# plainerman/DiffDock-Pocket

Hardware: AMD Instinct MI355X
Metric: ligand poses/sec (40 samples x 20 steps) on 3dpf (higher is better)
Workload: dtype f32 (fc and G products: fp16 hi/lo split of both operands on v_mfma_f32_16x16x32_f16 - the row-stationary conv kernel - and v_mfma_f32_32x32x16_f16, fp32 accumulate; G between its two kernels as fp16 hi + continuation byte = 19 significant bits; the exact fp32 MFMA form is timed in other_workloads)

## Files before the change

diffdock_pocket_amd/_lib.py:

```python
from __future__ import annotations

import ctypes as C
import operator
import os

HERE = os.path.dirname(os.path.abspath(__file__))
LIB_PATH = os.environ.get("DDP_HIP_LIB", os.path.join(HERE, "libddp_hip.so"))

DDP_MAX_TASKS, DDP_MAX_BLOCKS, DDP_MAX_SEGS, DDP_MAX_NS, DDP_EDGE_TILE = 9, 4, 3, 64, 64
F_SCALAR_S0, F_DOT, F_SCALAR_S1, F_VEC_S0, F_CROSS = range(5)
FS = 68

DDP_MAX_GEMM_BATCH = 16
DDP_EVAL_MAX_ATOMS = 1024
DDP_GUIDANCE_MAX_TORSIONS = 1024
DDP_MINIMIZE_MAX_ATOMS, DDP_MINIMIZE_MAX_TORSIONS = 512, 4096
DDP_MINIMIZE_FLEX_MAX_MOVING, DDP_MINIMIZE_FLEX_MAX_BONDS, DDP_MINIMIZE_FLEX_MAX_STATE_BYTES = 256, 256, 47040
DDP_SCORE_GUIDANCE_FLEX_MAX_ATOMS, DDP_SCORE_GUIDANCE_FLEX_MAX_TORSIONS = DDP_MINIMIZE_MAX_ATOMS, DDP_GUIDANCE_MAX_TORSIONS
DDP_SCORE_GUIDANCE_FLEX_MAX_MOVING, DDP_SCORE_GUIDANCE_FLEX_MAX_BONDS = DDP_MINIMIZE_FLEX_MAX_MOVING, DDP_MINIMIZE_FLEX_MAX_BONDS
DDP_PAIRWISE_MAX_SAMPLES, DDP_CLUSTER_MAX_SAMPLES = 32768, 1024
EXPORTS = ["ddp_conv_messages", "ddp_conv_rows", "ddp_stage_a_gh", "ddp_stage_a_gh3", "ddp_segment_reduce", "ddp_edge_featurize", "ddp_edge_featurize_jobs", "ddp_torsion_sh", "ddp_stage_a", "ddp_stage_a_h2",
           "ddp_pose_update", "ddp_sidechain_update", "ddp_sde_update", "ddp_radius_count", "ddp_radius_fill", "ddp_knn", "ddp_group_by_key", "ddp_node_linear", "ddp_scan_jobs", "ddp_mark_jobs", "ddp_rowcopy_jobs", "ddp_select_jobs",
           "ddp_gather_rows", "ddp_clean_pair_maps", "ddp_flex_mark", "ddp_fallback_rowmap", "ddp_step_prologue", "ddp_trrot_head", "ddp_tor_head", "ddp_radius_search_jobs", "ddp_group_by_key_jobs", "ddp_set_occupancy_shaping", "ddp_pose_rmsd", "ddp_pose_contacts", "ddp_pose_pairwise_rmsd", "ddp_pose_cluster", "ddp_traj_record", "ddp_svgd_tau", "ddp_svgd_pairs", "ddp_svgd_rows", "ddp_refine_energy", "ddp_refine_direction", "ddp_refine_accept", "ddp_clash_guidance", "ddp_score_guidance", "ddp_score_guidance_flex", "ddp_pose_score", "ddp_pose_profile", "ddp_pose_minimize", "ddp_pose_minimize_flex", "ddp_pose_search", "ddp_pose_search_select", "ddp_pose_search_flex", "ddp_pocket_occupancy", "ddp_pocket_buriedness", "ddp_pocket_label", "ddp_conv_deal_tile", "ddp_abi_version", "ddp_last_error", "ddp_source_hash"]


class Seg(C.Structure):
    _fields_ = [("kind", C.c_int32), ("in_off", C.c_int32), ("count", C.c_int32)]


class Block(C.Structure):
    _fields_ = [("U", C.c_int32), ("n", C.c_int32), ("C", C.c_int32), ("out_off", C.c_int32), ("tile0", C.c_int32),
                ("ntiles", C.c_int32), ("nsub", C.c_int32), ("ups", C.c_int32), ("nseg", C.c_int32),
                ("seg", Seg * DDP_MAX_SEGS), ("g_slot", C.c_int32), ("g_col0", C.c_int32)]


class RoleSeg(C.Structure):
    _fields_ = [("block", C.c_int32), ("tile0", C.c_int32), ("tstride", C.c_int32), ("count", C.c_int32), ("round", C.c_int32)]


DDP_CONV32_WAVES, DDP_MAX_ROLE_SEGS = 4, 2


class ConvShape(C.Structure):
    _fields_ = [("f_in", C.c_int32), ("hid", C.c_int32), ("kp1", C.c_int32), ("hp", C.c_int32), ("hs", C.c_int32),
                ("nct1", C.c_int32), ("d_out", C.c_int32), ("nblocks", C.c_int32), ("fbuf_floats", C.c_int32),
                ("g_cols", C.c_int32 * 2), ("blk", Block * DDP_MAX_BLOCKS), ("nrounds", C.c_int32),
                ("nrole", C.c_int32 * DDP_CONV32_WAVES), ("role", (RoleSeg * DDP_MAX_ROLE_SEGS) * DDP_CONV32_WAVES)]


class ConvTask(C.Structure):
    _fields_ = [("x_src", C.c_void_p), ("ldx_src", C.c_int32), ("n_edges", C.c_int32), ("src", C.c_void_p),
                ("eid", C.c_void_p), ("sh", C.c_void_p), ("seg_ptr", C.c_void_p * DDP_MAX_SEGS),
                ("seg_idx", C.c_void_p * DDP_MAX_SEGS), ("seg_ld", C.c_int32 * DDP_MAX_SEGS),
                ("seg_n", C.c_int32 * DDP_MAX_SEGS), ("w1p", C.c_void_p), ("b1p", C.c_void_p), ("w2p", C.c_void_p),
                ("b2p", C.c_void_p), ("msg", C.c_void_p), ("g", C.c_void_p * 2),
                ("pos", C.c_void_p), ("n_edges_dev", C.c_void_p), ("w1h", C.c_void_p), ("w2h", C.c_void_p), ("h2_range_flag", C.c_void_p),
                ("wsh", C.c_void_p), ("bsp", C.c_void_p), ("gh", C.c_void_p * 2), ("gh_fmt", C.c_int32), ("rows_form", C.c_int32), ("rows_bias_k", C.c_int32), ("rows_seg0", C.c_int32), ("rows_seg1", C.c_int32), ("rows_nts", C.c_int32)]


class ReduceSrc(C.Structure):
    _fields_ = [("msg", C.c_void_p), ("rowptr", C.c_void_p), ("bn_scale", C.c_void_p), ("bn_shift", C.c_void_p),
                ("n_edges", C.c_int32), ("rowmap", C.c_void_p), ("n_edges_dev", C.c_void_p)]


DDP_MAX_NODE_JOBS, DDP_MAX_NODE_CAT = 8, 16
DDP_MAX_LIST_JOBS = 12
_P, _I = C.c_void_p, C.c_int32


class ScanJob(C.Structure):
    _fields_ = [("n", _I), ("n_dev", _P), ("flag", _P), ("val", _P), ("rowptr", _P), ("base", _I), ("excl", _P), ("excl2", _P),
                ("list", _P), ("total", _P)]


class MarkJob(C.Structure):
    _fields_ = [("idx", _P), ("n", _I), ("n_dev", _P), ("mask", _P)]


class RowcopyJob(C.Structure):
    _fields_ = [("n_rows", _I), ("keep", _P), ("old_rowptr", _P), ("new_rowptr", _P), ("inp", _P * 3), ("out", _P * 3)]


class SelectJob(C.Structure):
    _fields_ = [("n", _I), ("n_dev", _P), ("mask_a", _P), ("idx_a", _P), ("mask_b", _P), ("idx_b", _P), ("out_idx", _P),
                ("pay", _P * 4), ("pay_add", _I * 4), ("out", _P * 4), ("total", _P), ("block_count", _P), ("block_off", _P)]


class RadiusJob(C.Structure):
    _fields_ = [("x", _P), ("x_ptr", _P), ("y", _P), ("y_batch", _P), ("ny", _I), ("r", C.c_float), ("max_neighbors", _I),
                ("flags", _I), ("graph_div", _P), ("counts", _P), ("offsets", _P), ("base", _I), ("total", _P), ("out_query", _P),
                ("out_x", _P), ("capacity", _I), ("overflow", _P)]


class SdeArgs(C.Structure):
    _fields_ = [("score", _P * 4), ("z", _P * 4), ("out", _P * 4), ("n", _I * 4)]


class SvgdArgs(C.Structure):
    _fields_ = [("pos", _P), ("n", _I), ("n_lig", _I), ("n_tor", _I), ("dihedrals", _P), ("score", _P * 3), ("upd", _P * 3), ("gdt", _P),
                ("weight", C.c_float), ("w_rep", C.c_float), ("w_rot", C.c_float), ("w_tor", C.c_float), ("svgd_only", _I),
                ("tau", _P), ("tr_diff", _P), ("rot_diff", _P), ("tor_diff", _P), ("dist", _P)]


class RefineArgs(C.Structure):
    _fields_ = [("n_samples", _I), ("n", _I), ("m", _I), ("rec_stride", _I), ("n_tor", _I), ("pos", _P), ("anchor", _P), ("lig_radii", _P),
                ("rec", _P), ("rec_radii", _P), ("self_pairs", _P), ("overlap", C.c_double), ("restraint", C.c_double), ("energy", _P),
                ("grad", _P), ("bonds", _P), ("mask_rotate", _P), ("step", _P), ("tr", _P), ("rot", _P), ("tor", _P), ("trial", _P),
                ("trial_energy", _P), ("trial_grad", _P), ("accepted", _P), ("grow", C.c_double), ("shrink", C.c_double),
                ("step_max", C.c_double)]


class GuidanceArgs(C.Structure):
    _fields_ = [("n_samples", _I), ("n", _I), ("m", _I), ("rec_stride", _I), ("n_tor", _I), ("pos", _P), ("lig_radii", _P), ("rec", _P),
                ("rec_radii", _P), ("self_pairs", _P), ("bonds", _P), ("mask_rotate", _P), ("overlap", C.c_double), ("weight", _P),
                ("max_tr", C.c_double), ("max_rot", C.c_double), ("max_tor", C.c_double), ("upd", _P * 3), ("energy", _P), ("grad", _P)]


class ScoreForm(C.Structure):
    _fields_ = [(k, C.c_double) for k in ("cutoff", "gauss_offset", "gauss_width", "hydrophobic_good", "hydrophobic_bad", "hbond_good",
                                          "hbond_bad", "w_gauss", "w_repulsion", "w_hydrophobic", "w_hbond")]
    _read = operator.attrgetter(*(k for k, _ in _fields_))

    @classmethod
    def from_config(cls, config) -> "ScoreForm":
        return cls(*cls._read(config))


class ScoreArgs(C.Structure):
    _anonymous_ = ("form",)
    _fields_ = [("n_samples", _I), ("n", _I), ("m", _I), ("rec_stride", _I), ("pos", _P), ("lig_radii", _P), ("lig_flags", _P), ("rec", _P),
                ("rec_radii", _P), ("rec_flags", _P), ("self_pairs", _P), ("form", ScoreForm), ("tor_divisor", C.c_double), ("energy", _P),
                ("grad", _P)]


class ScoreGuidanceArgs(C.Structure):
    _anonymous_ = ("form",)
    _fields_ = [("n_samples", _I), ("n", _I), ("m", _I), ("rec_stride", _I), ("n_tor", _I), ("pos", _P), ("lig_radii", _P), ("lig_flags", _P),
                ("rec", _P), ("rec_radii", _P), ("rec_flags", _P), ("self_pairs", _P), ("bonds", _P), ("mask_rotate", _P), ("form", ScoreForm),
                ("weight", _P), ("max_tr", C.c_double), ("max_rot", C.c_double), ("max_tor", C.c_double), ("upd", _P * 3), ("energy", _P),
                ("grad", _P)]


class ScoreGuidanceFlexArgs(C.Structure):
    _anonymous_ = ("form",)
    _fields_ = ScoreGuidanceArgs._fields_[:-2] + [("n_mov", _I), ("n_sc", _I), ("n_sub", _I), ("reserved", _I), ("mov", _P), ("sc_edge_idx", _P),
                                                  ("sc_sub", _P), ("sc_map", _P), ("sc_pairs", _P), ("max_sc", C.c_double), ("upd_sc", _P),
                                                  ("energy", _P), ("grad_mov", _P)]


class ProfileArgs(C.Structure):
    _anonymous_ = ("form",)
    _fields_ = [("n_samples", _I), ("n", _I), ("m", _I), ("rec_stride", _I), ("n_res", _I), ("reserved", _I), ("pos", _P), ("lig_radii", _P),
                ("lig_flags", _P), ("rec", _P), ("rec_radii", _P), ("rec_flags", _P), ("res_ptr", _P), ("form", ScoreForm),
                ("contact_distance", C.c_double), ("profile", _P), ("bits", _P)]


class MinimizeArgs(C.Structure):
    _anonymous_ = ("form",)
    _fields_ = [("n_samples", _I), ("n", _I), ("m", _I), ("rec_stride", _I), ("n_tor", _I), ("iterations", _I), ("pos", _P), ("anchor", _P),
                ("lig_radii", _P), ("lig_flags", _P), ("rec", _P), ("rec_radii", _P), ("rec_flags", _P), ("self_pairs", _P), ("bonds", _P),
                ("mask_rotate", _P), ("form", ScoreForm), ("restraint", C.c_double), ("grow", C.c_double), ("shrink", C.c_double),
                ("step_max", C.c_double), ("step", _P), ("accepted", _P), ("energy_in", _P), ("energy_out", _P), ("history", _P), ("grad", _P)]


class MinimizeFlexArgs(C.Structure):
    _anonymous_ = ("form",)
    _fields_ = MinimizeArgs._fields_ + [("rec_anchor", _P), ("n_mov", _I), ("n_sc", _I), ("n_sub", _I), ("reserved", _I), ("mov", _P),
                                        ("sc_edge_idx", _P), ("sc_sub", _P), ("sc_map", _P), ("sc_pairs", _P),
                                        ("restraint_sc", C.c_double), ("grad_mov", _P)]


class SearchArgs(C.Structure):
    _fields_ = [("min", MinimizeArgs), ("replicas", _I), ("cycles", _I), ("cycle0", _I), ("reserved", _I), ("step_init", C.c_double),
                ("temperature", C.c_double), ("perturb", _P), ("u", _P), ("cur_pos", _P), ("cur_e", _P), ("best_pos", _P), ("best_e", _P),
                ("best_cycle", _P), ("accepted", _P), ("trace", _P), ("flags", _P), ("starts", _P)]


class SearchFlexArgs(C.Structure):
    _fields_ = [("flex", MinimizeFlexArgs), ("replicas", _I), ("cycles", _I), ("cycle0", _I), ("reserved", _I), ("step_init", C.c_double),
                ("temperature", C.c_double), ("perturb", _P), ("u", _P), ("cur_pos", _P), ("cur_mov", _P), ("cur_e", _P), ("best_pos", _P),
                ("best_mov", _P), ("best_e", _P), ("best_cycle", _P), ("accepted", _P), ("trace", _P), ("flags", _P), ("starts", _P),
                ("starts_mov", _P)]


class SearchSelectArgs(C.Structure):
    _fields_ = [("n_samples", _I), ("n", _I), ("replicas", _I), ("reserved", _I), ("best_pos", _P), ("best_e", _P), ("best_cycle", _P),
                ("pos_out", _P), ("energy_out", _P), ("replica_out", _P), ("cycle_out", _P)]


def flex_state_bytes(n: int, n_mov: int, n_sc: int) -> int:
    return 89 * n + 81 * n_mov + 4 * n_sc


class GroupJob(C.Structure):
    _fields_ = [("key", _P), ("n_items", _I), ("n_items_dev", _P), ("n_keys", _I), ("pay", _P * 3), ("rowptr", _P), ("perm", _P),
                ("out_key", _P), ("out", _P * 3), ("key_map", _P), ("scratch", _P)]



DDP_MAX_FEATURIZE_JOBS = 8


class FeaturizeJob(C.Structure):
    _fields_ = [("pos_a", _P), ("ia", _P), ("pos_b", _P), ("ib", _P), ("n_edges", _I), ("n_edges_dev", _P), ("offset", _P), ("k_rbf", _I),
                ("coeff", C.c_float), ("pre", _P), ("pre_idx", _P), ("ld_pre", _I), ("pre2", _P), ("n_pre2", _I), ("ld_pre2", _I),
                ("w1d", _P), ("w2", _P), ("b2", _P), ("ns", _I), ("out", _P), ("sh", _P)]


class _BondJob(C.Structure):
    _fields_ = [("pos", _P), ("b0", _P), ("b1", _P), ("n", _I), ("mid", _P), ("vec", _P)]


class _CopyJob(C.Structure):
    _fields_ = [("src", _P), ("dst", _P), ("n", _I)]


class PrologueArgs(C.Structure):
    _fields_ = [("t", _P * 4), ("t_stride", _I * 4), ("sig_min", C.c_float * 4), ("sig_max", C.c_float * 4), ("sigma", _P * 4),
                ("n_graphs", _I), ("cut", _P), ("cut_mul", C.c_float), ("cut_add", C.c_float), ("graph_emb", _P), ("sd", _I),
                ("emb_scale", C.c_float), ("freq", _P), ("lig_pos", _P), ("graph_ptr", _P), ("center", _P),
                ("bonds", _BondJob * 2), ("copy", _CopyJob * 2)]


class TrRotArgs(C.Structure):
    _fields_ = [("gp", _P), ("ld_gp", _I), ("n_graphs", _I), ("ns", _I), ("sd", _I), ("graph_emb", _P), ("w1", _P * 2), ("b1", _P * 2),
                ("w2", _P * 2), ("b2", _P * 2), ("sigma", _P * 2), ("so3_table", _P), ("so3_n", _I), ("so3_lo", C.c_float),
                ("so3_span", C.c_float), ("out", _P * 2)]


class TorArgs(C.Structure):
    _fields_ = [("h", _P), ("ld_h", _I), ("n_bonds", _I), ("ns", _I), ("w1", _P), ("w2", _P), ("sigma", _P), ("graph_of_bond", _P),
                ("torus_table", _P), ("torus_n", _I), ("torus_lo", C.c_float), ("torus_span", C.c_float), ("out", _P)]


class NodeJob(C.Structure):
    _fields_ = [("n_rows", C.c_int32), ("cat", C.c_void_p), ("ld_cat", C.c_int32), ("n_cat", C.c_int32), ("table", C.c_void_p),
                ("feat_off", C.c_int32 * DDP_MAX_NODE_CAT), ("emb_dim", C.c_int32), ("emb_mode", C.c_int32),
                ("dense", C.c_void_p * 2), ("ld_dense", C.c_int32 * 2), ("n_dense", C.c_int32 * 2),
                ("t", C.c_void_p), ("t_stride", C.c_int32), ("scale", C.c_float), ("freq", C.c_void_p),
                ("sig_emb", C.c_void_p), ("ld_sig", C.c_int32), ("sd", C.c_int32), ("sig_out", C.c_void_p), ("ld_sig_out", C.c_int32),
                ("w", C.c_void_p), ("bias", C.c_void_p),
                ("out", C.c_void_p), ("ld_out", C.c_int32), ("ncols", C.c_int32), ("zero_to", C.c_int32),
                ("add", C.c_void_p), ("ld_add", C.c_int32)]


def g_ld(hid: int, gcols: int) -> int:
    return (((hid + 3) // 4 * 4 + 1) * gcols + 31) // 32 * 32


class DdpError(RuntimeError):
    pass


_lib = None


def load():
    global _lib
    if _lib is not None:
        return _lib
    if not os.path.exists(LIB_PATH):
        raise DdpError(f"{LIB_PATH} not found: build it with `python -m diffdock_pocket_amd.build` "
                       f"(hipcc --offload-arch=gfx950); there is no fallback path")
    lib = C.CDLL(LIB_PATH)
    for name in EXPORTS:
        if not hasattr(lib, name):
            raise DdpError(f"{LIB_PATH} does not export {name}")
    lib.ddp_abi_version.restype = C.c_int
    lib.ddp_last_error.restype = C.c_char_p
    lib.ddp_conv_messages.argtypes = [C.POINTER(ConvShape), C.POINTER(ConvTask), C.c_int, C.c_void_p]
    lib.ddp_conv_messages.restype = C.c_int
    lib.ddp_conv_rows.argtypes = lib.ddp_conv_messages.argtypes
    lib.ddp_conv_rows.restype = C.c_int
    lib.ddp_segment_reduce.argtypes = [C.c_void_p, C.c_int, C.c_int, C.c_int, C.POINTER(ReduceSrc), C.c_int, C.c_int,
                                       C.c_int, C.c_int, C.c_void_p]
    lib.ddp_segment_reduce.restype = C.c_int
    lib.ddp_edge_featurize.argtypes = [C.c_void_p, C.c_void_p, C.c_void_p, C.c_void_p, C.c_int, C.c_void_p, C.c_void_p, C.c_int,
                                       C.c_float, C.c_void_p, C.c_void_p, C.c_int, C.c_void_p, C.c_int, C.c_int, C.c_void_p,
                                       C.c_void_p, C.c_void_p, C.c_int, C.c_void_p, C.c_void_p, C.c_void_p]
    lib.ddp_edge_featurize.restype = C.c_int
    lib.ddp_edge_featurize_jobs.argtypes = [C.POINTER(FeaturizeJob), C.c_int, C.c_void_p]
    lib.ddp_edge_featurize_jobs.restype = C.c_int
    lib.ddp_torsion_sh.argtypes = [C.c_void_p, C.c_void_p, C.c_void_p, C.c_int, C.c_void_p, C.c_void_p, C.c_void_p, C.c_int, C.c_int,
                                   C.c_void_p, C.c_void_p, C.c_int, C.c_void_p, C.c_void_p]
    lib.ddp_torsion_sh.restype = C.c_int
    lib.ddp_stage_a.argtypes = [C.c_void_p, C.c_int, C.c_int, C.c_void_p, C.c_void_p, C.c_int, C.POINTER(C.c_int32), C.c_int,
                                C.c_void_p, C.c_void_p, C.c_int, C.c_int, C.c_void_p, C.c_int, C.c_void_p]
    lib.ddp_stage_a.restype = C.c_int
    lib.ddp_stage_a_h2.argtypes = lib.ddp_stage_a.argtypes[:-1] + [C.c_void_p, C.c_void_p]
    lib.ddp_stage_a_h2.restype = C.c_int
    lib.ddp_stage_a_gh.argtypes = lib.ddp_stage_a_h2.argtypes[:-1] + [C.c_void_p, C.c_void_p]
    lib.ddp_stage_a_gh.restype = C.c_int
    lib.ddp_stage_a_gh3.argtypes = lib.ddp_stage_a_gh.argtypes
    lib.ddp_stage_a_gh3.restype = C.c_int
    lib.ddp_set_occupancy_shaping.argtypes = [C.c_int, C.c_int]
    lib.ddp_set_occupancy_shaping.restype = C.c_int
    lib.ddp_pose_update.argtypes = [C.c_void_p, C.c_int, C.c_int, C.c_void_p, C.c_void_p, C.c_void_p, C.c_int, C.c_void_p,
                                    C.c_void_p, C.c_void_p, C.c_void_p]
    lib.ddp_pose_update.restype = C.c_int
    lib.ddp_sidechain_update.argtypes = [C.c_void_p, C.c_int, C.c_int, C.c_void_p, C.c_int, C.c_void_p, C.c_void_p, C.c_void_p,
                                         C.c_void_p, C.c_void_p]
    lib.ddp_sidechain_update.restype = C.c_int
    lib.ddp_radius_count.argtypes = [C.c_void_p, C.c_void_p, C.c_void_p, C.c_void_p, C.c_int, C.c_float, C.c_int, C.c_int,
                                     C.c_void_p, C.c_void_p]
    lib.ddp_radius_count.restype = C.c_int
    lib.ddp_radius_fill.argtypes = [C.c_void_p, C.c_void_p, C.c_void_p, C.c_void_p, C.c_int, C.c_float, C.c_int, C.c_int,
                                    C.c_void_p, C.c_void_p, C.c_void_p, C.c_void_p]
    lib.ddp_radius_fill.restype = C.c_int
    lib.ddp_knn.argtypes = [C.c_void_p, C.c_void_p, C.c_void_p, C.c_int, C.c_int, C.c_void_p, C.c_void_p]
    lib.ddp_knn.restype = C.c_int
    lib.ddp_group_by_key.argtypes = [C.c_void_p, C.c_int, C.c_int] + [C.c_void_p] * 11
    lib.ddp_group_by_key.restype = C.c_int
    for name, job in (("ddp_scan_jobs", ScanJob), ("ddp_mark_jobs", MarkJob), ("ddp_rowcopy_jobs", RowcopyJob),
                      ("ddp_select_jobs", SelectJob), ("ddp_radius_search_jobs", RadiusJob), ("ddp_group_by_key_jobs", GroupJob)):
        getattr(lib, name).argtypes = [C.POINTER(job), C.c_int, C.c_void_p]
        getattr(lib, name).restype = C.c_int
    lib.ddp_sde_update.argtypes = [C.c_void_p, C.POINTER(SdeArgs), C.c_void_p]
    lib.ddp_sde_update.restype = C.c_int
    lib.ddp_gather_rows.argtypes = [C.c_void_p, C.c_int, C.c_void_p, C.c_int, C.c_void_p, C.c_void_p, C.c_int, C.c_int, C.c_void_p]
    lib.ddp_gather_rows.restype = C.c_int
    lib.ddp_clean_pair_maps.argtypes = [C.c_void_p, C.c_void_p, C.c_void_p, C.c_void_p, C.c_int, C.c_int, C.c_int, C.c_int, C.c_void_p,
                                        C.c_void_p, C.c_void_p]
    lib.ddp_clean_pair_maps.restype = C.c_int
    lib.ddp_flex_mark.argtypes = [C.c_void_p, C.c_void_p, C.c_int, C.c_void_p, C.c_void_p, C.c_int, C.c_int, C.c_int, C.c_int, C.c_int,
                                  C.c_void_p, C.c_void_p]
    lib.ddp_flex_mark.restype = C.c_int
    lib.ddp_fallback_rowmap.argtypes = [C.c_void_p, C.c_void_p, C.c_void_p, C.c_void_p, C.c_int, C.c_int, C.c_void_p, C.c_void_p]
    lib.ddp_fallback_rowmap.restype = C.c_int
    for name, st in (("ddp_step_prologue", PrologueArgs), ("ddp_trrot_head", TrRotArgs), ("ddp_tor_head", TorArgs)):
        getattr(lib, name).argtypes = [C.POINTER(st), C.c_void_p]
        getattr(lib, name).restype = C.c_int
    lib.ddp_node_linear.argtypes = [C.POINTER(NodeJob), C.c_int, C.c_void_p]
    lib.ddp_node_linear.restype = C.c_int
    lib.ddp_pose_rmsd.argtypes = [C.c_void_p, C.c_int, C.c_int, C.c_void_p, C.c_int, C.c_void_p, C.c_int, C.c_void_p, C.c_int,
                                  C.c_void_p, C.c_void_p, C.c_void_p]
    lib.ddp_pose_rmsd.restype = C.c_int
    lib.ddp_pose_contacts.argtypes = [C.c_void_p, C.c_int, C.c_int, C.c_void_p, C.c_void_p, C.c_int, C.c_int, C.c_void_p, C.c_float,
                                      C.c_void_p, C.c_void_p, C.c_void_p]
    lib.ddp_pose_contacts.restype = C.c_int
    lib.ddp_pose_pairwise_rmsd.argtypes = [C.c_void_p, C.c_int, C.c_int, C.c_void_p, C.c_int, C.c_void_p, C.c_int, C.c_void_p, C.c_void_p]
    lib.ddp_pose_pairwise_rmsd.restype = C.c_int
    lib.ddp_pose_cluster.argtypes = [C.c_void_p, C.c_int, C.c_void_p, C.c_float, C.c_void_p, C.c_void_p, C.c_void_p, C.c_void_p, C.c_void_p]
    lib.ddp_pose_cluster.restype = C.c_int
    lib.ddp_traj_record.argtypes = [C.c_void_p, C.c_int, C.c_int, C.c_void_p, C.c_void_p, C.c_int, C.c_void_p, C.c_int, C.c_void_p,
                                    C.c_int, C.c_void_p, C.c_void_p]
    lib.ddp_traj_record.restype = C.c_int
    for name in ("ddp_svgd_tau", "ddp_svgd_pairs", "ddp_svgd_rows"):
        getattr(lib, name).argtypes = [C.POINTER(SvgdArgs), C.c_void_p]
        getattr(lib, name).restype = C.c_int
    for name in ("ddp_refine_energy", "ddp_refine_direction", "ddp_refine_accept"):
        getattr(lib, name).argtypes = [C.POINTER(RefineArgs), C.c_void_p]
        getattr(lib, name).restype = C.c_int
    lib.ddp_clash_guidance.argtypes = [C.POINTER(GuidanceArgs), C.c_void_p]
    lib.ddp_clash_guidance.restype = C.c_int
    lib.ddp_score_guidance.argtypes = [C.POINTER(ScoreGuidanceArgs), C.c_void_p]
    lib.ddp_score_guidance.restype = C.c_int
    lib.ddp_score_guidance_flex.argtypes = [C.POINTER(ScoreGuidanceFlexArgs), C.c_void_p]
    lib.ddp_score_guidance_flex.restype = C.c_int
    lib.ddp_pose_score.argtypes = [C.POINTER(ScoreArgs), C.c_void_p]
    lib.ddp_pose_score.restype = C.c_int
    lib.ddp_pose_profile.argtypes = [C.POINTER(ProfileArgs), C.c_void_p]
    lib.ddp_pose_profile.restype = C.c_int
    lib.ddp_pose_minimize.argtypes = [C.POINTER(MinimizeArgs), C.c_void_p]
    lib.ddp_pose_minimize.restype = C.c_int
    lib.ddp_pose_minimize_flex.argtypes = [C.POINTER(MinimizeFlexArgs), C.c_void_p]
    lib.ddp_pose_minimize_flex.restype = C.c_int
    lib.ddp_pose_search.argtypes = [C.POINTER(SearchArgs), C.c_void_p]
    lib.ddp_pose_search.restype = C.c_int
    lib.ddp_pose_search_select.argtypes = [C.POINTER(SearchSelectArgs), C.c_void_p]
    lib.ddp_pose_search_select.restype = C.c_int
    lib.ddp_pose_search_flex.argtypes = [C.POINTER(SearchFlexArgs), C.c_void_p]
    lib.ddp_pose_search_flex.restype = C.c_int
    lib.ddp_pocket_occupancy.argtypes = [C.c_void_p, C.c_void_p, C.c_int, C.c_float, C.c_float, C.c_float, C.c_float, C.c_int, C.c_int, C.c_int,
                                         C.c_void_p, C.c_void_p]
    lib.ddp_pocket_occupancy.restype = C.c_int
    lib.ddp_pocket_buriedness.argtypes = [C.c_void_p, C.c_int, C.c_int, C.c_int, C.c_double, C.c_double, C.c_int, C.c_void_p, C.c_void_p,
                                          C.c_void_p]
    lib.ddp_pocket_buriedness.restype = C.c_int
    lib.ddp_pocket_label.argtypes = [C.c_void_p, C.c_int, C.c_int, C.c_int, C.c_void_p, C.c_void_p]
    lib.ddp_pocket_label.restype = C.c_int
    lib.ddp_conv_deal_tile.argtypes = [C.c_int, C.c_int, C.c_int]
    lib.ddp_conv_deal_tile.restype = C.c_int
    if lib.ddp_abi_version() != 17:
        raise DdpError("libddp_hip.so ABI version mismatch")
    lib.ddp_source_hash.restype = C.c_char_p
    if "DDP_HIP_LIB" not in os.environ:
        from .build import source_hash
        have, want = lib.ddp_source_hash().decode(), source_hash()
        if have != want:
            raise DdpError(f"{LIB_PATH} was built from other sources (library {have}, tree {want}): rebuild it with "
                           f"`python -m diffdock_pocket_amd.build`")
    _lib = lib
    return lib


def check(rc, what):
    if rc != 0:
        raise DdpError(f"{what} failed (rc={rc}): {load().ddp_last_error().decode()}")
```

diffdock_pocket_amd/build.py:

```python
import hashlib
import os
import re
import subprocess
import sys
from concurrent.futures import ThreadPoolExecutor

HERE = os.path.dirname(os.path.abspath(__file__))
ROOT = os.path.dirname(HERE)
SOURCES = ["ddp_conv.hip", "ddp_conv_rows.hip", "ddp_conv_rows16.hip", "ddp_misc.hip", "ddp_gemm.hip", "ddp_pose.hip", "ddp_graph.hip", "ddp_views.hip", "ddp_lists.hip", "ddp_node.hip", "ddp_heads.hip",
           "ddp_eval.hip", "ddp_traj.hip", "ddp_svgd.hip", "ddp_refine.hip", "ddp_guidance.hip", "ddp_score_guidance.hip", "ddp_score_guidance_flex.hip", "ddp_score.hip", "ddp_profile.hip", "ddp_minimize.hip", "ddp_minimize_flex.hip", "ddp_search.hip", "ddp_search_flex.hip", "ddp_pockets.hip", "ddp_capi.hip"]
HEADERS = [os.path.join(HERE, "csrc", "ddp_internal.h"), os.path.join(HERE, "csrc", "ddp_conv_diag.h"), os.path.join(HERE, "csrc", "ddp_conv_common.h"), os.path.join(HERE, "csrc", "ddp_conv_deal.h"), os.path.join(HERE, "csrc", "ddp_conv_rows_common.h"), os.path.join(HERE, "csrc", "ddp_horn.h"), os.path.join(HERE, "csrc", "ddp_pockets_uf.h"), os.path.join(HERE, "csrc", "ddp_score_pair.h"), os.path.join(HERE, "csrc", "ddp_pose_descent.h"), os.path.join(HERE, "csrc", "ddp_minimize_loop.h"), os.path.join(HERE, "csrc", "ddp_minimize_flex_loop.h"), os.path.join(HERE, "csrc", "ddp_clash_energy.h"),
           os.path.join(ROOT, "include", "ddp_hip.h")]
OUT = os.path.join(HERE, "libddp_hip.so")
OBJ_DIR = os.path.join(HERE, "csrc", ".obj")
_TAG = re.compile(rb"DDP_SRC_SHA16=([0-9a-f]{16})")


def _deps():
    return [os.path.join(HERE, "csrc", s) for s in SOURCES] + [h for h in HEADERS if os.path.exists(h)]


def source_hash():
    h = hashlib.sha256()
    for d in _deps():
        h.update(os.path.basename(d).encode() + b"\0")
        with open(d, "rb") as f:
            h.update(f.read())
    return h.hexdigest()[:16]


def built_hash(path=None):
    path = path or OUT
    try:
        with open(path, "rb") as f:
            m = _TAG.search(f.read())
    except OSError:
        return None
    return m.group(1).decode() if m else None


def needs_build():
    return built_hash() != source_hash()


EXTRA_FLAGS = {"ddp_conv_rows.hip": [] if os.environ.get("DDP_ROWS_SLP") else ["-fno-slp-vectorize"],
               "ddp_conv_rows16.hip": [] if os.environ.get("DDP_ROWS_SLP") else ["-fno-slp-vectorize"]}


def _compile(src, flags, verbose):
    flags = list(flags) + EXTRA_FLAGS.get(src, [])
    path = os.path.join(HERE, "csrc", src)
    h = hashlib.sha256(" ".join(flags).encode())
    for d in [path] + [x for x in HEADERS if os.path.exists(x)]:
        with open(d, "rb") as f:
            h.update(f.read())
    os.makedirs(OBJ_DIR, exist_ok=True)
    obj = os.path.join(OBJ_DIR, f"{os.path.splitext(src)[0]}.{h.hexdigest()[:16]}.o")
    if not os.path.exists(obj):
        for old in os.listdir(OBJ_DIR):
            if old.startswith(os.path.splitext(src)[0] + ".") and len(os.listdir(OBJ_DIR)) > 64:
                os.remove(os.path.join(OBJ_DIR, old))
        cmd = [os.environ.get("HIPCC", "hipcc"), "--offload-arch=gfx950", "-O3", "-std=c++17", "-fPIC", "-c"] + flags + \
              ["-I", os.path.join(ROOT, "include"), "-I", os.path.join(HERE, "csrc"), "-o", obj + ".tmp", path]
        if verbose:
            print(" ".join(cmd), flush=True)
        subprocess.check_call(cmd)
        os.replace(obj + ".tmp", obj)
    return obj


def _link(out, defs, verbose):
    sha = f'-DDDP_SRC_SHA16="{source_hash()}"'
    flags = [f"-D{d}" for d in defs]
    with ThreadPoolExecutor(max_workers=min(4, os.cpu_count() or 1)) as ex:
        objs = list(ex.map(lambda s: _compile(s, flags + ([sha] if s == "ddp_capi.hip" else []), verbose), SOURCES))
    cmd = [os.environ.get("HIPCC", "hipcc"), "--offload-arch=gfx950", "-shared", "-fPIC", "-o", out + ".tmp"] + objs
    if verbose:
        print(" ".join(cmd), flush=True)
    subprocess.check_call(cmd)
    os.replace(out + ".tmp", out)
    return out


def build(force=False, verbose=True, stamps=False, ablate=0, defs=(), tag=""):
    if defs:
        return _link(os.path.join(HERE, f"libddp_hip_{tag}.so"), list(defs), verbose)
    if ablate or stamps:
        out = os.path.join(HERE, "libddp_hip" + ("_stamps" if stamps else "") + (f"_ablate{ablate}" if ablate else "") + ".so")
        return _link(out, (["DDP_STAMPS"] if stamps else []) + ([f"DDP_ABLATE={ablate}"] if ablate else []), verbose)
    if not force and not needs_build():
        return OUT
    return _link(OUT, [], verbose)


if __name__ == "__main__":
    build(force="--force" in sys.argv, stamps="--stamps" in sys.argv)
```

diffdock_pocket_amd/csrc/ddp_graph.hip:

```cpp
#include <hip/hip_runtime.h>
#include <stdint.h>

#include "ddp_hip.h"
#include "ddp_internal.h"

#define DDP_KNN_MAX 32

__device__ __forceinline__ float sqdist(const float* __restrict__ a, const float* __restrict__ b) {
#pragma clang fp contract(off)
  const float dx = a[0] - b[0], dy = a[1] - b[1], dz = a[2] - b[2];
  const float xx = dx * dx, yy = dy * dy, zz = dz * dz;
  return (xx + yy) + zz;
}

__device__ __forceinline__ void load_pt(const float* __restrict__ p, size_t j, bool scaled, float div, float out[3]) {
  out[0] = p[3 * j];
  out[1] = p[3 * j + 1];
  out[2] = p[3 * j + 2];
  if (scaled) {
    out[0] = __fdiv_rn(out[0], div);
    out[1] = __fdiv_rn(out[1], div);
    out[2] = __fdiv_rn(out[2], div);
  }
}

__device__ __forceinline__ float sqdist_to(const float* __restrict__ yq, const float* __restrict__ x, size_t j, bool scaled, float div) {
  float xj[3];
  load_pt(x, j, scaled, div, xj);
  return sqdist(yq, xj);
}

#define DDP_CUT_LIST 64
__device__ float radius_cut(const float* __restrict__ x, int j0, int j1, const float* __restrict__ yq, float r2, int cap, bool scaled,
                            float div) {
  if (cap <= DDP_CUT_LIST) {
    float best[DDP_CUT_LIST];
#pragma unroll
    for (int i = 0; i < DDP_CUT_LIST; ++i) best[i] = __builtin_inff();
    float worst = __builtin_inff();
    for (int j = j0; j < j1; ++j) {
      float d = sqdist_to(yq, x, (size_t)j, scaled, div);
      if (!(d < r2) || !(d < worst)) continue;
      bool shifting = false;
#pragma unroll
      for (int i = 0; i < DDP_CUT_LIST; ++i) {
        if (i < cap && (shifting || d < best[i])) {
          const float t = best[i];
          best[i] = d;
          d = t;
          shifting = true;
        }
        if (i == cap - 1) worst = best[i];
      }
    }
    return worst;
  }
  float cut = r2;
  for (int i = j0; i < j1; ++i) {
    const float di = sqdist_to(yq, x, (size_t)i, scaled, div);
    if (!(di < r2) || !(di < cut)) continue;
    int le = 0;
    for (int j = j0; j < j1; ++j) {
      const float dj = sqdist_to(yq, x, (size_t)j, scaled, div);
      le += (dj < r2 && dj <= di) ? 1 : 0;
    }
    if (le >= cap) cut = di;
  }
  return cut;
}

struct RadiusLaunch {
  int njobs;
  int blk_start[DDP_MAX_LIST_JOBS + 1];
  ddp_radius_job_t job[DDP_MAX_LIST_JOBS];
};

template <bool FILL>
__global__ __launch_bounds__(256) void ddp_radius_kernel(const RadiusLaunch L) {
  int jb_ = 0;
  while (jb_ + 1 < L.njobs && (int)blockIdx.x >= L.blk_start[jb_ + 1]) ++jb_;
  const ddp_radius_job_t& J = L.job[jb_];
  const int q = ((int)blockIdx.x - L.blk_start[jb_]) * 4 + ((int)threadIdx.x >> 6), lane = (int)threadIdx.x & 63;
  if (q >= J.ny) return;
  if (FILL && !J.out_x) return;
  const float* __restrict__ x = J.x;
  const int g = J.y_batch[q];
  const int j0 = J.x_ptr[g], j1 = J.x_ptr[g + 1];
  const bool scaled = J.graph_div != nullptr;
  const float div = scaled ? J.graph_div[g] : 1.f;
  const float r2 = J.r * J.r;
  const int cap = J.max_neighbors, flags = J.flags;
  float yq[3];
  load_pt(J.y, (size_t)q, scaled, div, yq);
  int n = 0;
  for (int j = j0 + lane; j < j1; j += 64) n += (sqdist_to(yq, x, (size_t)j, scaled, div) < r2) ? 1 : 0;
#pragma unroll
  for (int m = 32; m > 0; m >>= 1) n += __shfl_xor(n, m);
  const bool drop_self = (flags & DDP_RADIUS_DROP_SELF) != 0, nearest = (flags & DDP_RADIUS_NEAREST) != 0;
  float lim = r2;
  bool capped = false;
  if (n > cap && nearest) {
    float c = 0.f;
    if (lane == 0) c = radius_cut(x, j0, j1, yq, r2, cap, scaled, div);
    lim = __shfl(c, 0);
    capped = true;
  }
  int kept = 0, seen = 0;
  const int obase = FILL ? J.offsets[q] : 0;
  for (int jb = j0; jb < j1; jb += 64) {
    const int j = jb + lane;
    bool match = false;
    if (j < j1) {
      const float d = sqdist_to(yq, x, (size_t)j, scaled, div);
      match = capped ? (d < r2 && d <= lim) : (d < r2);
    }
    const unsigned long long mm = __ballot(match);
    if (!nearest) match = match && (seen + __popcll(mm & ((1ull << lane) - 1ull)) < cap);
    seen += __popcll(mm);
    const bool ok = match && !(drop_self && j == q);
    const unsigned long long mk = __ballot(ok);
    if (FILL && ok) {
      const int o = obase + kept + __popcll(mk & ((1ull << lane) - 1ull));
      if (o < J.capacity) {
        J.out_query[o] = q;
        J.out_x[o] = j;
      } else if (J.overflow) {
        *J.overflow = 1;
      }
    }
    kept += __popcll(mk);
    if (!nearest && seen >= cap) break;
  }
  if (!FILL && lane == 0) J.counts[q] = kept;
}

__global__ __launch_bounds__(256) void ddp_knn_kernel(const float* __restrict__ x, const int32_t* __restrict__ x_ptr,
                                                      const int32_t* __restrict__ batch, int n, int k,
                                                      int32_t* __restrict__ out_nb ) {
  const int q = blockIdx.x * 4 + (threadIdx.x >> 6), lane = threadIdx.x & 63;
  if (q >= n) return;
  const int g = batch[q];
  const int j0 = x_ptr[g], j1 = x_ptr[g + 1];
  const float yq[3] = {x[3 * (size_t)q], x[3 * (size_t)q + 1], x[3 * (size_t)q + 2]};
  const int none = 0x7fffffff;
  float pd = -1.f;
  int pj = -1;
  constexpr int CAP = 24;
  if (j1 - j0 <= 64 * CAP) {
    float dl[CAP];
#pragma unroll
    for (int c = 0; c < CAP; ++c) {
      const int j = j0 + lane + 64 * c;
      float d = __builtin_inff();
      if (j < j1 && j != q) d = sqdist(yq, x + 3 * (size_t)j);
      dl[c] = (d < __builtin_inff()) ? d : __builtin_inff();
    }
    for (int t = 0; t < k; ++t) {
      float bd = __builtin_inff();
      int bj = none;
#pragma unroll
      for (int c = 0; c < CAP; ++c) {
        const int j = j0 + lane + 64 * c;
        const float d = dl[c];
        const bool after = (d > pd) || (d == pd && j > pj);
        if (d < __builtin_inff() && after && (d < bd || (d == bd && j < bj))) { bd = d; bj = j; }
      }
#pragma unroll
      for (int off = 32; off >= 1; off >>= 1) {
        const float od = __shfl_xor(bd, off);
        const int oj = __shfl_xor(bj, off);
        if (od < bd || (od == bd && oj < bj)) { bd = od; bj = oj; }
      }
      if (bj == none) {
        for (int u = t + lane; u < k; u += 64) out_nb[(size_t)q * k + u] = -1;
        return;
      }
      if (lane == 0) out_nb[(size_t)q * k + t] = bj;
      pd = bd;
      pj = bj;
    }
    return;
  }
  for (int t = 0; t < k; ++t) {
// ... 109 lines not shown
```

diffdock_pocket_amd/engine.py:

```python
from __future__ import annotations

import ctypes as C
from collections.abc import Mapping
from types import SimpleNamespace
from typing import Dict, List, Optional

import math

import torch

from . import _lib as L
from . import graph as G
from . import launch as K
from . import packing as P
from . import packing as P_
from .graph import EdgeView

SRC_TYPE = {0: "l", 1: "r", 2: "a", 3: "a", 4: "l", 5: "r", 6: "r", 7: "l", 8: "a"}
RECV_TYPE = {0: "l", 1: "l", 2: "l", 3: "a", 4: "a", 5: "a", 6: "r", 7: "r", 8: "r"}
RECV_OF = {"a": (3, 4, 5), "r": (6, 7, 8)}
ORDER = {"l": [0, 2, 1], "a": [3, 4, 5], "r": [6, 8, 7]}
_DROP_SELF = 1


class LazyStats(Mapping):

    def __init__(self, static: Dict[str, int], counts: Optional[K.CountBlock], names: Dict[str, str]):
        self._static, self._counts, self._names, self._vals = dict(static), counts, dict(names), None

    def _resolve(self):
        if self._vals is None:
            vals = dict(self._static)
            if self._counts is not None:
                host = self._counts.values()
                for key, slot in self._names.items():
                    if slot in host:
                        vals[key] = host[slot]
            self._vals = vals
        return self._vals

    def fresh(self):
        return LazyStats(self._static, self._counts, self._names)

    def __getitem__(self, k):
        return self._resolve()[k]

    def __iter__(self):
        return iter(self._resolve())

    def __len__(self):
        return len(self._resolve())


def _i32(t):
    return t.to(torch.int32).contiguous()


def direct_packs(convs, dev):
    packs = []
    for conv, nsplit in convs:
        pkr = conv.packed_rows_direct(dev, nsplit)
        packs.append([] if pkr is None else (pkr if nsplit > 1 else [pkr]))
    if all(pks and all(K.conv_path(pk).rows for pk in pks) for pks in packs):
        return packs
    return [[conv.packed(dev)] for conv, _ in convs]


class _Fork:

    def __init__(self, dev, n):
        self.main = torch.cuda.current_stream(dev)
        self.side = [torch.cuda.Stream(device=dev) for _ in range(n)]
        self.used = []

    def run(self, i, fn):
        st = self.side[i % len(self.side)]
        if st not in self.used:
            st.wait_stream(self.main)
            self.used.append(st)
        with torch.cuda.stream(st):
            return fn()

    def resync(self, i):
        st = self.side[i % len(self.side)]
        if st in self.used:
            st.wait_stream(self.main)

    def join(self, only=None):
        for st in list(self.used):
            if only is None or st is self.side[only % len(self.side)]:
                self.main.wait_stream(st)
                self.used.remove(st)


class ForwardEngine:
    def __init__(self, model):
        self.m = model
        self._forks = {}

    def _fork(self, dev):
        f = self._forks.get(dev)
        if f is None:
            f = self._forks[dev] = _Fork(dev, 5)
        f.main = torch.cuda.current_stream(dev)
        return f

    @torch.no_grad()
    def forward(self, data):
        lig = data["ligand"]
        K.require_hip(lig.pos)
        with torch.cuda.device(lig.pos.device):
            return self._forward(data)

    def _forward(self, data):
        m = self.m
        lig, rec, atom = data["ligand"], data["receptor"], data["atom"]
        dev = lig.pos.device
        m._refresh_weight_caches()
        m.rows_all_or_none(dev)
        m.check_overflow(range_too=m.range_check_in_forward)
        K.CONV_H2 = m.conv_h2
        if dev in self._forks:
            self._forks[dev].used.clear()
        K.set_range_flag(m.overflow_flag(dev)[1:2])
        mark = m.section_timer.mark if m.section_timer is not None else (lambda name: None)
        mark("start")
        if m.no_aminoacid_identities:
            rec.x = rec.x * 0
        S = self._static(data, lig, rec, atom, dev)
        ff = None
        if (m.fork_front and m.section_timer is None and m.before_layers is None and m.debug_conv_outputs is None
                and not m.exact_sizes):
            ff = self._fork(dev)
        F = self._front(data, S, lig, rec, atom, dev, mark, ff)
        F.lists_fork = ff
        self._lists(S, F, dev, side=(lambda fn: ff.run(4, fn)) if ff is not None else None)
        mark("lists")
        if m.exact_sizes:
            self._exact(F)
        if m.before_layers is not None:
            m.before_layers()
        self._layers(S, F, dev, mark)
        out = self._heads(data, S, F, lig, rec, atom, dev, mark)
        m.last_stats = LazyStats(S.stats, F.cnt, {"E_ll": "ll", "E_lr": "lr", "E_la": "la", "n_near": "near",
                                                  "clean1_dirty_edges": "dirty", "flex0_kept_aa_edges": "fx_3"})
        prof = K.profiler()
        if prof is not None:
            prof.hold = getattr(prof, "hold", [])
            prof.hold.append(F.cnt.block)
        return out

    def _static(self, data, lig, rec, atom, dev):
        m = self.m
        S = SimpleNamespace()
        B = S.B = int(data.num_graphs)
        lbatch, rbatch, abatch = lig.batch.long(), rec.batch.long(), atom.batch.long()
        S.lbatch, S.rbatch, S.abatch = lbatch, rbatch, abatch
        S.Nl, S.Nr, S.Na = lig.pos.shape[0], rec.pos.shape[0], atom.pos.shape[0]
        S.lay_l = m._cached("lay_l", (lig.batch,), lambda: G.DenseLayout.build(lbatch, B))
        S.lay_r = m._cached("lay_r", (rec.batch,), lambda: G.DenseLayout.build(rbatch, B))
        S.lay_a = m._cached("lay_a", (atom.batch,), lambda: G.DenseLayout.build(abatch, B))
        for lay in (S.lay_l, S.lay_r, S.lay_a):
            G._ptr(lay)
        bond_ei = data["ligand", "ligand"].edge_index
        S.bond_ei = bond_ei
        S.bond32 = m._cached("bond32", (bond_ei,), lambda: (_i32(bond_ei[0]), _i32(bond_ei[1])))
        S.E_bond = int(bond_ei.shape[1])
        rr, ar = data["receptor", "receptor"].edge_index, data["atom", "receptor"].edge_index
        S.rr, S.ar = rr, ar
        S.num_flex = 0
        if m.flexible_sidechains and len(data["flexResidues"]) > 0:
            S.num_flex = int(data["flexResidues"].edge_idx.shape[0])
        nl, nr, na = S.lay_l.counts_host, S.lay_r.counts_host, S.lay_a.counts_host
        S.cap_ll = S.E_bond + sum(n * min(max(n - 1, 0), 33) for n in nl)
        S.cap_lr = sum(a * min(b, 10000) for a, b in zip(nl, nr))
        S.cap_la = sum(a * min(b, 10000, max(int(m.la_capacity_per_atom), 1)) for a, b in zip(nl, na))
        S.stats = {"E_rr": int(rr.shape[1]), "E_ar": int(ar.shape[1]), "N_l": S.Nl, "N_r": S.Nr, "N_a": S.Na, "B": B}
        S.tor = S.sc = None
        if not m.confidence_mode:
            if not m.no_torsion:
                def tor_static():
                    idx = lig.edge_mask.bool().nonzero(as_tuple=True)[0]
                    bnd = bond_ei[:, idx].long()
                    bb = lbatch[bnd[0]]
                    lay = G.DenseLayout.build(bb, B) if idx.shape[0] > 0 else None
                    return SimpleNamespace(idx=idx, bonds=bnd, batch=bb, lay=lay, T=int(idx.shape[0]), flat32=_i32(bnd.reshape(-1)),
                                           batch32=_i32(bb))
                tor = m._cached("tor_static", (lig.edge_mask, bond_ei, lig.batch), tor_static)
                if tor.T > 0:
                    G._ptr(tor.lay)
                    tor.cap = sum(t * min(n, 32) for t, n in zip(tor.lay.counts_host, nl))
                    S.tor = tor
            if S.num_flex > 0:
                fr = data["flexResidues"]

                def sc_static():
                    sb = fr.batch.long()
                    bonds = S.lay_a.starts[sb] + fr.edge_idx.t().long()
                    return SimpleNamespace(bonds=bonds, batch=sb, lay=G.DenseLayout.build(sb, B), T=int(sb.shape[0]),
                                           flat32=_i32(bonds.reshape(-1)), batch32=_i32(sb))
                sc = m._cached("sc_static", (fr.batch, fr.edge_idx, atom.batch), sc_static)
                G._ptr(sc.lay)
                sc.cap = sum(t * min(n, 32) for t, n in zip(sc.lay.counts_host, na))
                S.sc = sc
        return S

    def _one_time(self, data, lig, rec, atom):
        ts = (rec.node_t["tr"], atom.node_t["tr"])
        if all(t.numel() > 0 and (t.numel() == 1 or t.stride(0) == 0) for t in ts) and ts[0].data_ptr() == ts[1].data_ptr():
            return True
        hint = getattr(data, "ddp_time_hint", None)
        if hint is not None and hint[0] == tuple(id(t) for t in ts) and hint[1] == tuple(t._version for t in ts):
            return bool(hint[2])
        t_nodes = torch.cat([t.reshape(-1) for t in ts])
        return bool((t_nodes == t_nodes[0]).all().item()) if t_nodes.numel() else True

    @staticmethod
    def _smooth_weight(pos_a, idx_a, pos_b, idx_b, max_norm):
        ia = idx_a.long().clamp(0, pos_a.shape[0] - 1)
        ib = idx_b.long().clamp(0, pos_b.shape[0] - 1)
        d = (pos_b[ib] - pos_a[ia]).norm(dim=-1)
        return 0.5 * (torch.cos(torch.clip(d * math.pi / max_norm, max=math.pi)) + 1.0)

    def _prologue(self, data, S, F, lig, dev, ll0, ll1):
        m = self.m
        B = S.B
        a = L.PrologueArgs()
        ts = [data.complex_t[k] for k in ("tr", "rot", "tor", "sc_tor")]
        ts = [t if t.dtype == torch.float32 else t.float() for t in ts]
        keep = [ts]
        a.n_graphs = B
        for k, t in enumerate(ts):
            a.t[k], a.t_stride[k] = K._p(t), (t.stride(0) if t.numel() > 1 else 0)
        rng = None if m.confidence_mode else m._sigma_ranges()
        if m.confidence_mode:
            F.sig = [t.expand(B).contiguous() for t in ts]
        elif rng is None:
            F.sig = [s.float().expand(B).contiguous() for s in m.t_to_sigma(*ts)]
        else:
            sig = torch.empty((4, B), device=dev)
            F.sig = [sig[k] for k in range(4)]
            for k in range(4):
                a.sig_min[k], a.sig_max[k] = rng[k]
        for k in range(4):
            a.sigma[k] = K._p(F.sig[k])
        F.cut = None
        if m.dynamic_max_cross:
            F.cut = torch.empty(B, device=dev)
            a.cut, a.cut_mul, a.cut_add = K._p(F.cut), 3.0, 20.0
        F.center = F.graph_emb = None
        if not m.confidence_mode:
            spec = m._sigma_spec(ts[0], dev)
            if spec[0] == "t":
                F.graph_emb = torch.empty((B, spec[4]), device=dev)
                a.graph_emb, a.sd, a.emb_scale, a.freq = K._p(F.graph_emb), spec[4], spec[2], K._p(spec[3])
            else:
                F.graph_emb = spec[1]
            keep.append(spec)
            F.center = torch.empty((B, 3), device=dev)
            a.lig_pos, a.graph_ptr, a.center = K._p(F.lpos), K._p(S.lay_l._ptr32), K._p(F.center)
        F.tor = F.sc = None
        for i, (name, st, pos) in enumerate((("tor", S.tor, F.lpos), ("sc", S.sc, F.apos))):
            if st is None:
                continue
            h = SimpleNamespace(st=st, bond_pos=torch.empty((st.T, 3), device=dev), bond_vec=torch.empty((st.T, 3), device=dev))
            b = a.bonds[i]
            b.pos, b.b0, b.b1, b.n = K._p(pos), K._p(st.flat32[:st.T]), K._p(st.flat32[st.T:]), st.T
            b.mid, b.vec = K._p(h.bond_pos), K._p(h.bond_vec)
            setattr(F, name, h)
        for i, (src, dst) in enumerate(((S.bond32[0], ll0), (S.bond32[1], ll1))):
            a.copy[i].src, a.copy[i].dst, a.copy[i].n = K._p(src), K._p(dst), S.E_bond
        L.check(L.load().ddp_step_prologue(C.byref(a), K.stream()), "ddp_step_prologue")
        F.keep_pro = (keep, a)

    def _front(self, data, S, lig, rec, atom, dev, mark, ff=None):
        m = self.m
        ns, B = m.ns, S.B
        F = SimpleNamespace()
        cnt = F.cnt = K.CountBlock(dev)
        lpos, rpos, apos = lig.pos.float().contiguous(), rec.pos.float().contiguous(), atom.pos.float().contiguous()
        F.lpos, F.rpos, F.apos = lpos, rpos, apos
        Nl, Nr, Na = S.Nl, S.Nr, S.Na
        lay_l, lay_r, lay_a = S.lay_l, S.lay_r, S.lay_a
        i32e = lambda n: torch.empty(n, dtype=torch.int32, device=dev)
        Eb = S.E_bond
        ll0, ll1 = i32e(S.cap_ll), i32e(S.cap_ll)
        self._prologue(data, S, F, lig, dev, ll0, ll1)

        nt = (lambda: m._node_tables(lig, rec, atom, dev))
        F.xl, F.xr, F.xa, pre = ff.run(0, nt) if ff is not None else nt()
        F.pre = pre
        mark("node_embed")
        sd_, dd, cd, nf = m.sigma_embed_dim, m.distance_embed_dim, m.cross_distance_embed_dim, m.in_lig_edge_features
        epk = {}
        for key, name, rbf0, rbf_n in (("ll", "lig_edge_embedding", nf + sd_, dd), ("rr", "rec_edge_embedding", sd_, dd),
                                       ("aa", "atom_edge_embedding", sd_, dd), ("lr", "lr_edge_embedding", sd_, cd),
                                       ("la", "la_edge_embedding", sd_, cd), ("ar", "ar_edge_embedding", sd_, dd)):
            epk[key] = m._edge_pack(name, slice(rbf0, rbf0 + rbf_n), dev)
        bond_attr = data["ligand", "ligand"].edge_attr
        bond_pre = m._cached("bond_pre", (bond_attr,), lambda: (bond_attr.float() @ epk["ll"].W1[:, :nf].t()).contiguous())

        ptr_l, ptr_r, ptr_a = lay_l._ptr32, lay_r._ptr32, lay_a._ptr32
        b32_l, b32_r, b32_a = G._batch32(lay_l, Nl), G._batch32(lay_r, Nr), G._batch32(lay_a, Na)
        rr = S.rr
        kk = m.atom_max_neighbors if m.atom_max_neighbors else 32
        aa = m._cached("aa", (atom.pos, atom.batch), lambda: G.knn_graph(apos, kk, lay_a))
        data["atom", "atom"].edge_index = aa
        F.aa = aa
        S.stats["E_aa"] = int(aa.shape[1])
        lr0, lr1, la0, la1 = i32e(S.cap_lr), i32e(S.cap_lr), i32e(S.cap_la), i32e(S.cap_la)
        jobs = [K.radius_job(lpos, ptr_l, lpos, b32_l, m.lig_max_radius, 33, _DROP_SELF, i32e(Nl), i32e(Nl + 1), base=Eb,
                             total=cnt["ll"], out_query=ll1, out_x=ll0, capacity=S.cap_ll)]
        cut = None
        if m.dynamic_max_cross:
            cut = F.cut
            jobs.append(K.radius_job(rpos, ptr_r, lpos, b32_l, 1.0, 10000, 0, i32e(Nl), i32e(Nl + 1), total=cnt["lr"],
                                     out_query=lr0, out_x=lr1, capacity=S.cap_lr, graph_div=cut))
        else:
            jobs.append(K.radius_job(rpos, ptr_r, lpos, b32_l, m.cross_max_distance, 10000, 0, i32e(Nl), i32e(Nl + 1), total=cnt["lr"],
                                     out_query=lr0, out_x=lr1, capacity=S.cap_lr))
        jobs.append(K.radius_job(apos, ptr_a, lpos, b32_l, m.lig_max_radius, 10000, 0, i32e(Nl), i32e(Nl + 1), total=cnt["la"],
                                 out_query=la0, out_x=la1, capacity=S.cap_la, overflow=m.overflow_flag(dev)))
        F.touched = i32e(Na)
        jobs.append(K.radius_job(lpos, ptr_l, apos, b32_a, m.lig_max_radius, 10000, 0, F.touched))
        for name, st, pos, ptr_x in (("tor", S.tor, lpos, ptr_l), ("sc", S.sc, apos, ptr_a)):
            if st is None:
                continue
            h = getattr(F, name)
            h.q, h.x = i32e(st.cap), i32e(st.cap)
            jobs.append(K.radius_job(pos, ptr_x, h.bond_pos, G._batch32(st.lay, st.T), m.lig_max_radius, 32, 0, i32e(st.T),
                                     i32e(st.T + 1), total=cnt[name], out_query=h.q, out_x=h.x, capacity=st.cap))
            setattr(F, name, h)
        K.radius_search_jobs(jobs)
        F.keep = [jobs, cut]
        F.near_rows = i32e(Na)
        K.scan_jobs([K.scan_job(Na, flag=F.touched, lst=F.near_rows, total=cnt["near"])])
        mark("searches")

        shared0 = {}
        if m.share_layer0 and B > 1 and m.debug_conv_outputs is None and self._one_time(data, lig, rec, atom):
            ar = S.ar
            if S.num_flex > 0:
                sh_ = m._cached("shared0_rec", (rec.x, rec.pos, rr, atom.x, ar),
                                lambda: m._shared_receptor_side(B, rec, atom, rpos, apos, lay_r, lay_a, rr.long(), ar.long(), aa, atoms="static"))
            else:
                sh_ = m._cached("shared0", (rec.x, rec.pos, atom.x, atom.pos, rr, ar, aa),
                                lambda: m._shared_receptor_side(B, rec, atom, rpos, apos, lay_r, lay_a, rr.long(), ar.long(), aa))
            shared0 = {k: v for k, v in sh_.items() if v is not None}
        F.flex_static = shared0.pop("flex", None)
        F.shared0 = shared0

        def rows32(name, ei, k):
            r0, r1 = m._cached(name, (ei,), lambda: (_i32(ei[0]), _i32(ei[1])))
            n = shared0[k][1] if k in shared0 else ei.shape[1]
            return r0[:n], r1[:n]

        rr32, aa32, ar32 = rows32("rr32", rr, 6), rows32("aa32", aa, 3), rows32("ar32", S.ar, 5)

        F.e, F.sh = {}, {}
        calls = {
            "ll": ((epk["ll"], m.lig_distance_expansion, lpos, ll0, lpos, ll1, pre["ll"], ll0), dict(pre2=bond_pre, n_edges=S.cap_ll, cnt=cnt["ll"])),
            "rr": ((epk["rr"], m.rec_distance_expansion, rpos, rr32[0], rpos, rr32[1], pre["rr"], rr32[0]), {}),
            "aa": ((epk["aa"], m.lig_distance_expansion, apos, aa32[0], apos, aa32[1], pre["aa"], aa32[0]), {}),
            "lr": ((epk["lr"], m.cross_distance_expansion, lpos, lr0, rpos, lr1, pre["lr"], lr0), dict(n_edges=S.cap_lr, cnt=cnt["lr"])),
            "la": ((epk["la"], m.cross_distance_expansion, lpos, la0, apos, la1, pre["la"], la0), dict(n_edges=S.cap_la, cnt=cnt["la"])),
            "ar": ((epk["ar"], m.rec_distance_expansion, apos, ar32[0], rpos, ar32[1], pre["ar"], ar32[0]), {})}
        def feat():
            res = K.edge_featurize_jobs(list(calls.values()))
            if m.smooth_edges:
                cut_e = (lambda: F.cut[b32_l.long()[lr0.long().clamp(0, Nl - 1)]]) if m.dynamic_max_cross else (lambda: m.cross_max_distance)
                for key, mx in (("ll", m.lig_max_radius), ("rr", m.rec_max_radius), ("aa", m.lig_max_radius), ("lr", None), ("la", m.lig_max_radius)):
                    (_, _, pa, ia, pb, ib, _, _), _ = calls[key]
                    sh_k = res[list(calls).index(key)][1]
                    if sh_k.shape[0] > 0:
                        sh_k.mul_(self._smooth_weight(pa, ia[:sh_k.shape[0]], pb, ib[:sh_k.shape[0]], cut_e() if mx is None else mx).unsqueeze(1))
            return res
        if ff is not None:
            ff.resync(0)
        for key, (o_, s_) in zip(calls, ff.run(0, feat) if ff is not None else feat()):
            F.e[key], F.sh[key] = o_, s_
        mark("edge_featurize")

        def static_csr(name, k, ei, recv, src, n):
            if k in shared0:
                e0 = shared0[k][1]

                def modded():
                    c = G.build_csr(recv, src, n)
                    return G.CSR(c.n_edges, c.recv, c.src, (c.eid % e0).contiguous(), c.rowptr)
                return m._cached(f"{name}_mod{e0}", (ei,), modded)
            return m._cached(name, (ei,), lambda: G.build_csr(recv, src, n))

        c = {}
        g1 = []
        aa_per_step = S.num_flex > 0 and aa.shape[1] > 0
        if aa_per_step:
            v = SimpleNamespace(rp=i32e(Na + 1), perm=i32e(aa.shape[1]), key=i32e(aa.shape[1]), o0=i32e(aa.shape[1]))
            g1.append(K.group_job(aa32[0], aa.shape[1], Na, [aa32[1]], v.rp, v.perm, v.key, [v.o0], i32e(Na + aa.shape[1])))
            c[3] = G.CSR(int(aa.shape[1]), v.key, v.o0, v.perm, v.rp)
        else:
            c[3] = static_csr("c_aa", 3, aa, aa[0], aa[1], Na)
        c[5] = static_csr("c_ar", 5, S.ar, S.ar[0], S.ar[1], Na)
        c[6] = static_csr("c_rr", 6, rr, rr[0], rr[1], Nr)
        c[8] = static_csr("c_ra", 8, S.ar, S.ar[1], S.ar[0], Nr)
        v = SimpleNamespace(rp=i32e(Nl + 1), perm=i32e(S.cap_ll), key=i32e(S.cap_ll), o0=i32e(S.cap_ll))
        g1.append(K.group_job(ll0, S.cap_ll, Nl, [ll1], v.rp, v.perm, v.key, [v.o0], i32e(Nl + S.cap_ll), n_dev=cnt["ll"]))
        c[0] = EdgeView(S.cap_ll, v.key, v.o0, v.perm, rowptr=v.rp, cnt=cnt["ll"])
        for k, q0, x1, cap, name in ((1, lr0, lr1, S.cap_lr, "lr"), (2, la0, la1, S.cap_la, "la")):
            rp = i32e(Nl + 1)
            g1.append(K.group_job(q0, cap, Nl, [], rp, scratch=i32e(Nl), n_dev=cnt[name]))
            c[k] = EdgeView(cap, q0, x1, G.iota32(cap, dev), rowptr=rp, cnt=cnt[name])
        for k, key, pay, cap, n_keys, name in ((4, la1, la0, S.cap_la, Na, "la"), (7, lr1, lr0, S.cap_lr, Nr, "lr")):
            v = SimpleNamespace(rp=i32e(n_keys + 1), perm=i32e(cap), key=i32e(cap), o0=i32e(cap))
            g1.append(K.group_job(key, cap, n_keys, [pay], v.rp, v.perm, v.key, [v.o0], i32e(n_keys + cap), n_dev=cnt[name]))
            c[k] = EdgeView(cap, v.key, v.o0, v.perm, rowptr=v.rp, cnt=cnt[name])
        for h, name in ((F.tor, "tor"), (F.sc, "sc")):
            if h is not None:
                h.rp = i32e(h.st.T + 1)
                g1.append(K.group_job(h.q, h.st.cap, h.st.T, [], h.rp, scratch=i32e(h.st.T), n_dev=cnt[name]))
                h.csr = EdgeView(h.st.cap, h.q, h.x, G.iota32(h.st.cap, dev), rowptr=h.rp, cnt=cnt[name])
        K.group_jobs(g1)
        F.keep.append(g1)
        F.c = c
        n_src = {"l": Nl, "a": Na, "r": Nr}
        so = {}
        F.fact = set()
        if m.factorize_min_degree > 0:
            F.fact = {0, 1, 2, 3, 4, 5, 6, 7}
            for k in (3, 5, 6):
                if k == 3 and aa_per_step:
                    continue
                so[k] = m._cached(f"so_{k}", (c[k].src, c[k].eid), lambda k=k: G.source_order(c[k], n_src[SRC_TYPE[k]]))
            so[1] = EdgeView(S.cap_lr, c[7].src, c[7].recv, c[7].eid, pos=c[7].eid, cnt=cnt["lr"])
            so[2] = EdgeView(S.cap_la, c[4].src, c[4].recv, c[4].eid, pos=c[4].eid, cnt=cnt["la"])
            g2 = []
            if aa_per_step:
                E3 = c[3].n_edges
                v = SimpleNamespace(rp=i32e(Na + 1), perm=i32e(E3), key=i32e(E3), o0=i32e(E3), o1=i32e(E3))
                g2.append(K.group_job(c[3].src, E3, Na, [c[3].recv, c[3].eid], v.rp, v.perm, v.key, [v.o0, v.o1], i32e(Na + E3)))
                so[3] = G.SourceOrder(E3, v.o0, v.key, v.o1, v.perm)
            for k, cap, name in ((0, S.cap_ll, "ll"), (4, S.cap_la, "la"), (7, S.cap_lr, "lr")):
                v = SimpleNamespace(rp=i32e(Nl + 1), perm=i32e(cap), key=i32e(cap), o0=i32e(cap), o1=i32e(cap))
                g2.append(K.group_job(c[k].src, cap, Nl, [c[k].recv, c[k].eid], v.rp, v.perm, v.key, [v.o0, v.o1], i32e(Nl + cap),
                                      n_dev=cnt[name]))
                so[k] = EdgeView(cap, v.o0, v.key, v.o1, pos=v.perm, cnt=cnt[name])
            K.group_jobs(g2)
            F.keep.append(g2)
        F.so = so
        if ff is not None:
            ff.join(only=0)
        mark("views")
        return F

    def _lists(self, S, F, dev, side=None):
        m = self.m
        L_, B = m.num_conv_layers, S.B
        Nl, Nr, Na = S.Nl, S.Nr, S.Na
        cnt, c, so = F.cnt, F.c, F.so
        i32e = lambda n: torch.empty(n, dtype=torch.int32, device=dev)
        zpool = [torch.zeros(6 * (Na + Nr) + Na + 64, dtype=torch.int32, device=dev), 0]
        F.keep.append(zpool)

        def i32z(n):
            if zpool[1] + n > zpool[0].numel():
                return torch.zeros(n, dtype=torch.int32, device=dev)
            v = zpool[0][zpool[1]:zpool[1] + n]
            zpool[1] += (n + 3) & ~3
            return v
        F.pruned, F.pruned_so, F.rows_a = {}, {}, {}
        F.clean1 = None
        n_of = {"l": Nl, "a": Na, "r": Nr}
        dbg = m.debug_conv_outputs is not None
        E_aa = c[3].n_edges

        def prune():
            prune_on = (m.prune_last_receptor_layer and L_ >= 2 and not m.confidence_mode and not dbg and E_aa >= m.plan_min_edges
                        and not (m.flexible_sidechains and F.sc is None))
            if prune_on:
                layers = [l for l in (L_ - 1, L_ - 2) if l >= 1 and (l != L_ - 1 or m.flexible_sidechains)]
                need = {"a": i32z(Na), "r": i32z(Nr)}
                if F.sc is not None:
                    K.mark_jobs([K.mark_job(need["a"], F.sc.st.flat32, 2 * F.sc.st.T),
                                 K.mark_job(need["a"], F.sc.csr.src, F.sc.csr.n_edges, cnt["sc"])])
                else:
                    K.mark_jobs([K.mark_job(need["a"], c[2].src, c[2].n_edges, cnt["la"]),
                                 K.mark_job(need["r"], c[1].src, c[1].n_edges, cnt["lr"])])
                for l in layers:
                    act = {"a": m.flexible_sidechains or l != L_ - 1}
                    act["r"] = act["a"] and l != L_ - 1
                    scans, copies, pl = [], [], {}
                    for rt in ("a", "r"):
                        if not act[rt]:
                            continue
                        for k in RECV_OF[rt]:
                            full = c[k]
                            if full.n_edges == 0:
                                continue
                            name = f"p{l}_{k}"
                            n = n_of[rt]
                            v = EdgeView(full.n_edges, i32e(full.n_edges), i32e(full.n_edges), i32e(full.n_edges), rowptr=i32e(n + 1), cnt=cnt[name])
                            scans.append(K.scan_job(n, flag=need[rt], rowptr=full.rowptr, excl=v.rowptr, total=cnt[name]))
                            copies.append(K.rowcopy_job(n, need[rt], full.rowptr, v.rowptr, [full.recv, full.src, full.eid], [v.recv, v.src, v.eid]))
                            pl[k] = v
                    K.scan_jobs(scans)
                    K.rowcopy_jobs(copies)
                    F.pruned[l] = pl
                    rows_mask = {"a": i32z(Na), "r": i32z(Nr)}
                    marks = []
                    for k in range(9):
                        rt, st_ = RECV_TYPE[k], SRC_TYPE[k]
                        if st_ == "l" or k == 2 or k not in F.fact or (rt != "l" and not act[rt]):
                            continue
                        vw = pl.get(k, c[k])
                        if vw.n_edges > 0:
                            marks.append(K.mark_job(rows_mask[st_], vw.src, vw.n_edges, vw.cnt))
                    nxt = None
                    if l != layers[-1]:
                        nxt = {"a": need["a"].clone(), "r": need["r"].clone()}
                        for k in range(9):
                            rt, st_ = RECV_TYPE[k], SRC_TYPE[k]
                            if st_ == "l" or (rt != "l" and not act[rt]):
                                continue
                            vw = pl.get(k, c[k])
                            if vw.n_edges > 0:
                                marks.append(K.mark_job(nxt[st_], vw.src, vw.n_edges, vw.cnt))
                    K.mark_jobs(marks)
                    lists = {}
                    scans = []
                    for t in ("a", "r"):
                        rows = i32e(n_of[t])
                        scans.append(K.scan_job(n_of[t], flag=rows_mask[t], lst=rows, total=cnt[f"rows{l}_{t}"]))
                        lists[t] = (rows, cnt[f"rows{l}_{t}"])
                    K.scan_jobs(scans)
                    F.rows_a[l] = lists
                    if nxt is not None:
                        need = nxt
                gj = []
                for l, pl in F.pruned.items():
                    for k, v in pl.items():
                        if k in F.fact:
                            n_keys = n_of[SRC_TYPE[k]]
                            w = SimpleNamespace(rp=i32e(n_keys + 1), perm=i32e(v.n_edges), key=i32e(v.n_edges), o0=i32e(v.n_edges), o1=i32e(v.n_edges))
                            gj.append(K.group_job(v.src, v.n_edges, n_keys, [v.recv, v.eid], w.rp, w.perm, w.key, [w.o0, w.o1],
                                                  i32e(n_keys + v.n_edges), n_dev=v.cnt))
                            F.pruned_so.setdefault(l, {})[k] = EdgeView(v.n_edges, w.o0, w.key, w.o1, pos=w.perm, cnt=v.cnt)
                K.group_jobs(gj)
                F.keep.append(gj)

        def flex0():
            F.flex0 = None
            fx = getattr(F, "flex_static", None)
            kk = m.atom_max_neighbors if m.atom_max_neighbors else 32
            if (fx is not None and m.share_flex_layer0 and S.num_flex > 0 and not dbg and 0 not in F.pruned and L_ >= 2
                    and 3 in F.fact and 5 in F.fact and E_aa == Na * kk and E_aa % B == 0 and E_aa >= m.plan_min_edges
                    and E_aa * m.ns >= m.flex_share_min_work):
                na, e_ar, nr = fx
                e0 = E_aa // B
                qdirty, dirty, need_r = i32z(Na), i32z(Na), i32z(Nr)
                K.flex_mark(c[3].src, c[3].recv, E_aa, e0, na, na, qdirty, pos=F.apos, a_too=True, ref_list=True)
                K.flex_mark(c[3].recv, c[3].src, E_aa, e0, na, na, dirty, flag=qdirty, a_too=True, ref_list=True)
                K.flex_mark(c[8].recv, c[8].src, c[8].n_edges, e_ar, nr, na, need_r, pos=F.apos)
                scans, copies, pl, rowmaps = [], [], {}, {}
                for k, need, n in ((3, dirty, Na), (5, dirty, Na), (8, need_r, Nr)):
                    full = c[k]
                    v = EdgeView(full.n_edges, i32e(full.n_edges), i32e(full.n_edges), i32e(full.n_edges), rowptr=i32e(n + 1), cnt=cnt[f"fx_{k}"])
                    scans.append(K.scan_job(n, flag=need, rowptr=full.rowptr, excl=v.rowptr, total=cnt[f"fx_{k}"]))
                    copies.append(K.rowcopy_job(n, need, full.rowptr, v.rowptr, [full.recv, full.src, full.eid], [v.recv, v.src, v.eid]))
                    pl[k] = v
                K.scan_jobs(scans)
                K.rowcopy_jobs(copies)
                for k, need, n_per in ((3, dirty, na), (5, dirty, na), (8, need_r, nr)):
                    rowmaps[k] = i32e(c[k].n_edges)
                    K.fallback_rowmap(need, c[k].recv, c[k].rowptr, pl[k].rowptr, c[k].n_edges, n_per, rowmaps[k])
                rows_mask = {"a": i32z(Na), "r": i32z(Nr)}
                marks = [K.mark_job(rows_mask["a"], pl[3].src, pl[3].n_edges, pl[3].cnt),
                         K.mark_job(rows_mask["r"], pl[5].src, pl[5].n_edges, pl[5].cnt)]
                if 1 in F.fact and c[1].n_edges > 0:
                    marks.append(K.mark_job(rows_mask["r"], c[1].src, c[1].n_edges, c[1].cnt))
                K.mark_jobs(marks)
                lists, scans = {}, []
                for t in ("a", "r"):
                    rows = i32e(n_of[t])
                    scans.append(K.scan_job(n_of[t], flag=rows_mask[t], lst=rows, total=cnt[f"rows0_{t}"]))
                    lists[t] = (rows, cnt[f"rows0_{t}"])
                K.scan_jobs(scans)
                gj, pso = [], {}
                for k in (3, 5):
                    v = pl[k]
                    n_keys = n_of[SRC_TYPE[k]]
                    w = SimpleNamespace(rp=i32e(n_keys + 1), perm=i32e(v.n_edges), key=i32e(v.n_edges), o0=i32e(v.n_edges), o1=i32e(v.n_edges))
                    gj.append(K.group_job(v.src, v.n_edges, n_keys, [v.recv, v.eid], w.rp, w.perm, w.key, [w.o0, w.o1],
                                          i32e(n_keys + v.n_edges), n_dev=v.cnt))
                    pso[k] = EdgeView(v.n_edges, w.o0, w.key, w.o1, pos=w.perm, cnt=v.cnt)
                K.group_jobs(gj)
                F.keep.append(gj)
                F.pruned[0], F.pruned_so[0], F.rows_a[0] = pl, pso, lists
                F.flex0 = SimpleNamespace(dirty=dirty, need_r=need_r, rowmaps=rowmaps, na=na, e0=e0)
# ... 481 lines not shown
```

diffdock_pocket_amd/launch.py:

```python
from __future__ import annotations

import ctypes as C
import os
from dataclasses import dataclass
from typing import Dict, List, NamedTuple, Optional, Sequence

import torch
from torch import nn

from . import _lib as L
from . import packing as P
from .graph import EdgeView


def require_hip(t: torch.Tensor):
    if not t.is_cuda:
        raise L.DdpError("the MI355X score model runs on a HIP device only (no CPU/eager fallback); "
                         "move the batch to cuda:<n>")
    L.load()


def stream():
    return C.c_void_p(torch._C._cuda_getCurrentRawStream(torch._C._cuda_getDevice()))

# ... 318 lines not shown
        j.pre2, j.n_pre2, j.ld_pre2 = (_p(pre2) if n2 else 0), n2, (pre2.stride(0) if n2 else 0)
        j.w1d, j.w2, j.b2, j.ns, j.out, j.sh = _p(pack.w1d), _p(pack.w2), _p(pack.b2), pack.ns, _p(out), _p(sh)
        jobs.append(j)
        keep.append((pre, pre2, ia, ib, pre_idx))
    if jobs:
        arr = (L.FeaturizeJob * len(jobs))(*jobs)
        L.check(L.load().ddp_edge_featurize_jobs(arr, len(jobs), stream()), "ddp_edge_featurize_jobs")
    return outs


@dataclass
class StageAStack:
    W: torch.Tensor
    meta: list
    offs: object
    path: ConvPath
    gh: Optional[torch.Tensor]
    ld: int
    Wh: Optional[torch.Tensor] = None
    W3: Optional[torch.Tensor] = None

    def prepare(self, h2: bool, x3: bool) -> "StageAStack":
        if (h2 or self.path.rows) and self.Wh is None:
            self.Wh = P.split_h2(self.W, unified_scale=P.GH_SW) if self.path.rows else P.split_h2(self.W)
        if x3 and not self.path.rows and self.W3 is None:
            self.W3 = P.split_bf16x3(self.W)
        return self


def stage_a_stack(packs, hid: int, path: ConvPath) -> StageAStack:
    Ws, meta, ghs, lds = [], [], [], set()
    for key, pk in packs:
        for slot in (0, 1):
            if pk.wg[slot] is None:
                continue
            meta.append((key, slot, pk.g_in_off[slot]))
            Ws.append(pk.wgh[slot] if path.rows else pk.wg[slot])
            if path.rows:
                ghs.append(pk.gh_groups[slot])
                lds.add(pk.gh_ld[slot])
    assert len(lds) <= 1, "the convs of one stage-A launch write G rows of one length"
    W = torch.stack(Ws).contiguous()
    gh = torch.stack([P.gh_dest_table(ws, (hid + 7) // 8, W.shape[2], fmt=path.gh_fmt) for ws in ghs]).contiguous().to(W.device) if path.rows else None
    return StageAStack(W, meta, (C.c_int32 * len(meta))(*[mm[2] for mm in meta]), path, gh, lds.pop() if lds else W.shape[2])


def stage_a(x, n_rows, st: StageAStack, out, rows=None, rows_cnt=None, out_rows=None, h2=False, x3=False):
    lib = L.load()
    nb, n_in, ncols = st.W.shape
    if nb > L.DDP_MAX_GEMM_BATCH:
        raise L.DdpError("more (conv, slot) pairs per source array than DDP_MAX_GEMM_BATCH")
    if n_rows == 0:
        return
    args = (x.data_ptr(), x.stride(0), n_rows, ptr(rows), ptr(rows_cnt), out_rows if out_rows is not None else n_rows, st.offs, nb,
            st.W.data_ptr())
    if st.path.rows:
        fn, name = (lib.ddp_stage_a_gh3, "ddp_stage_a_gh3") if st.path.gh_fmt == 1 else (lib.ddp_stage_a_gh, "ddp_stage_a_gh")
        L.check(fn(*args, ptr(st.Wh), n_in, ncols, out.data_ptr(), st.ld, ptr(_RANGE_FLAG), st.gh.data_ptr(), stream()), name)
    elif h2:
        L.check(lib.ddp_stage_a_h2(*args, ptr(st.Wh), n_in, ncols, out.data_ptr(), ncols, ptr(_RANGE_FLAG), stream()), "ddp_stage_a_h2")
    else:
        L.check(lib.ddp_stage_a(*args, ptr(st.W3 if x3 else None), n_in, ncols, out.data_ptr(), ncols, stream()), "ddp_stage_a")


def _hold(j, *objs):
    j._keep = objs
    return j


def _run_jobs(fn, cls, jobs, what):
    lib = L.load()
    for i in range(0, len(jobs), L.DDP_MAX_LIST_JOBS):
        part = jobs[i:i + L.DDP_MAX_LIST_JOBS]
        arr = (cls * len(part))(*part)
        L.check(getattr(lib, fn)(arr, len(part), stream()), what)


def scan_job(n, flag=None, val=None, rowptr=None, base=0, excl=None, excl2=None, lst=None, total=None, n_dev=None) -> L.ScanJob:
    j = L.ScanJob()
    j.n, j.n_dev, j.flag, j.val, j.rowptr, j.base = n, _p(n_dev), _p(flag), _p(val), _p(rowptr), base
    j.excl, j.excl2, j.list, j.total = _p(excl), _p(excl2), _p(lst), _p(total)
    return _hold(j, flag, val, rowptr, excl, excl2, lst, total, n_dev)


def scan_jobs(jobs: Sequence[L.ScanJob]):
    _run_jobs("ddp_scan_jobs", L.ScanJob, list(jobs), "ddp_scan_jobs")


def mark_job(mask, idx, n, n_dev=None) -> L.MarkJob:
    j = L.MarkJob()
    j.idx, j.n, j.n_dev, j.mask = _p(idx), n, _p(n_dev), _p(mask)
    return _hold(j, idx, n_dev, mask)


def mark_jobs(jobs: Sequence[L.MarkJob]):
    _run_jobs("ddp_mark_jobs", L.MarkJob, list(jobs), "ddp_mark_jobs")


def rowcopy_job(n_rows, keep, old_rowptr, new_rowptr, ins, outs) -> L.RowcopyJob:
    j = L.RowcopyJob()
    j.n_rows, j.keep, j.old_rowptr, j.new_rowptr = n_rows, _p(keep), _p(old_rowptr), _p(new_rowptr)
    for k, (a, b) in enumerate(zip(ins, outs)):
        j.inp[k], j.out[k] = _p(a), _p(b)
    return _hold(j, keep, old_rowptr, new_rowptr, list(ins), list(outs))


def rowcopy_jobs(jobs: Sequence[L.RowcopyJob]):
    _run_jobs("ddp_rowcopy_jobs", L.RowcopyJob, list(jobs), "ddp_rowcopy_jobs")


def select_job(n, mask_a, idx_a, mask_b, idx_b, pays, outs, total, scratch, out_idx=None, n_dev=None, pay_add=None) -> L.SelectJob:
    j = L.SelectJob()
    nb = (n + 2047) // 2048
    j.n, j.n_dev, j.mask_a, j.idx_a, j.mask_b, j.idx_b, j.out_idx = n, _p(n_dev), _p(mask_a), _p(idx_a), _p(mask_b), _p(idx_b), _p(out_idx)
    for k, (a, b) in enumerate(zip(pays, outs)):
        j.pay[k], j.out[k] = _p(a), _p(b)
        j.pay_add[k] = 0 if pay_add is None else pay_add[k]
    j.total = _p(total)
    j.block_count, j.block_off = scratch.data_ptr(), scratch.data_ptr() + 4 * nb
    return _hold(j, n_dev, mask_a, idx_a, mask_b, idx_b, out_idx, list(pays), list(outs), total, scratch)


def select_jobs(jobs: Sequence[L.SelectJob]):
    _run_jobs("ddp_select_jobs", L.SelectJob, list(jobs), "ddp_select_jobs")


def radius_job(x, x_ptr, y, y_batch, r, cap, flags, counts, offsets=None, base=0, total=None, out_query=None, out_x=None,
               capacity=0, graph_div=None, overflow=None) -> L.RadiusJob:
    j = L.RadiusJob()
    j.x, j.x_ptr, j.y, j.y_batch, j.ny = x.data_ptr(), x_ptr.data_ptr(), y.data_ptr(), y_batch.data_ptr(), int(y.shape[0])
    j.r, j.max_neighbors, j.flags, j.graph_div = float(r), int(cap), int(flags), _p(graph_div)
    j.counts, j.offsets, j.base, j.total = _p(counts), _p(offsets), int(base), _p(total)
    j.out_query, j.out_x, j.capacity, j.overflow = _p(out_query), _p(out_x), int(capacity), _p(overflow)
    return _hold(j, x, x_ptr, y, y_batch, graph_div, counts, offsets, total, out_query, out_x, overflow)


def radius_search_jobs(jobs: Sequence[L.RadiusJob]):
    _run_jobs("ddp_radius_search_jobs", L.RadiusJob, list(jobs), "ddp_radius_search_jobs")


def group_job(key, n_items, n_keys, pays, rowptr, perm=None, out_key=None, outs=(), scratch=None, n_dev=None, key_map=None) -> L.GroupJob:
    j = L.GroupJob()
    j.key, j.n_items, j.n_items_dev, j.n_keys = _p(key), n_items, _p(n_dev), n_keys
    for k, a in enumerate(pays):
        j.pay[k] = _p(a)
    j.rowptr, j.perm, j.out_key, j.key_map, j.scratch = _p(rowptr), _p(perm), _p(out_key), _p(key_map), _p(scratch)
    for k, a in enumerate(outs):
        j.out[k] = _p(a)
    return _hold(j, key, n_dev, list(pays), rowptr, perm, out_key, list(outs), key_map, scratch)


def group_jobs(jobs: Sequence[L.GroupJob]):
    _run_jobs("ddp_group_by_key_jobs", L.GroupJob, list(jobs), "ddp_group_by_key_jobs")


def gather_rows(x, idx, n, out, ncols, n_dev=None):
    lib = L.load()
    if n > 0:
        L.check(lib.ddp_gather_rows(x.data_ptr(), x.stride(0), idx.data_ptr(), n, ptr(n_dev), out.data_ptr(), out.stride(0), ncols,
                                    stream()), "ddp_gather_rows")


def flex_mark(a, b, n_edges, e0, n_a_per_graph, n_b_per_graph, mark, pos=None, flag=None, a_too=False, ref_list=False):
    L.check(L.load().ddp_flex_mark(ptr(pos), ptr(flag), n_b_per_graph, ptr(a), ptr(b), n_edges, e0, n_a_per_graph, int(a_too), int(ref_list),
                                   ptr(mark), stream()), "ddp_flex_mark")


def fallback_rowmap(mark, recv, old_rowptr, new_rowptr, n_edges, n_recv_per_graph, rowmap):
    L.check(L.load().ddp_fallback_rowmap(ptr(mark), ptr(recv), ptr(old_rowptr), ptr(new_rowptr), n_edges, n_recv_per_graph, ptr(rowmap),
                                         stream()), "ddp_fallback_rowmap")


def clean_pair_maps(touched, recv, src, n_edges, e0, n_graphs, n0, rowmap, rows_v, rowptr=None):
    lib = L.load()
    L.check(lib.ddp_clean_pair_maps(touched.data_ptr(), recv.data_ptr(), src.data_ptr(), ptr(rowptr), n_edges, e0, n_graphs, n0,
                                    rowmap.data_ptr(), rows_v.data_ptr(), stream()), "ddp_clean_pair_maps")


def _eval_arg(t, dtype, dev, what):
    if t.device != dev or t.dtype != dtype or not t.is_contiguous():
        raise L.DdpError(f"{what}: expected a contiguous {dtype} tensor on {dev}, got {t.dtype} on {t.device}")


def pose_rmsd(pred, ref, perms, sel=None, rmsd=None, best=None):
    dev = pred.device
    S, n, P = pred.shape[0], perms.shape[0], perms.shape[1]
    for t, dt, w in ((pred, torch.float32, "pred"), (ref, torch.float32, "ref"), (perms, torch.int32, "perms")):
        _eval_arg(t, dt, dev, f"pose_rmsd {w}")
    if sel is not None:
        _eval_arg(sel, torch.int32, dev, "pose_rmsd sel")
        if sel.shape != (n,):
            raise L.DdpError("pose_rmsd: sel must have one entry per perms row")
    elif n > pred.shape[1]:
        raise L.DdpError("pose_rmsd: more perms rows than pred rows")
    if pred.dim() != 3 or pred.shape[2] != 3 or ref.dim() != 2 or ref.shape[1] != 3 or perms.dim() != 2:
        raise L.DdpError("pose_rmsd: pred [S, rows, 3], ref [n_ref, 3], perms [n, P]")
    rmsd = torch.empty(S, dtype=torch.float32, device=dev) if rmsd is None else rmsd
    best = torch.empty(S, dtype=torch.int32, device=dev) if best is None else best
    if S == 0:
        return rmsd, best
    L.check(L.load().ddp_pose_rmsd(pred.data_ptr(), S, pred.shape[1] * 3, _p(sel), n, ref.data_ptr(), ref.shape[0], perms.data_ptr(), P,
                                   rmsd.data_ptr(), best.data_ptr(), stream()), "ddp_pose_rmsd")
    return rmsd, best


def pose_contacts(lig, lig_radii, rec, rec_radii, ref_centroid, overlap=0.4, out=None):
    dev = lig.device
    S, n = lig.shape[0], lig.shape[1]
    for t, w in ((lig, "lig"), (lig_radii, "lig_radii"), (rec, "rec"), (rec_radii, "rec_radii"), (ref_centroid, "ref_centroid")):
        _eval_arg(t, torch.float32, dev, f"pose_contacts {w}")
    if lig.dim() != 3 or lig.shape[2] != 3 or rec.dim() not in (2, 3) or rec.shape[-1] != 3:
        raise L.DdpError("pose_contacts: lig [S, n, 3], rec [m, 3] or [S, m, 3]")
    m = rec.shape[-2]
    if rec.dim() == 3 and rec.shape[0] != S:
        raise L.DdpError("pose_contacts: a per-sample receptor needs one row block per sample")
    if lig_radii.shape != (n,) or rec_radii.shape != (m,) or ref_centroid.numel() != 3:
        raise L.DdpError("pose_contacts: radii / centroid shapes")
    out = torch.empty(S, 4, dtype=torch.float32, device=dev) if out is None else out
    if S == 0:
        return out
    L.check(L.load().ddp_pose_contacts(lig.data_ptr(), S, n, lig_radii.data_ptr(), rec.data_ptr(), m, 3 * m if rec.dim() == 3 else 0,
                                       rec_radii.data_ptr(), float(overlap), ref_centroid.data_ptr(), out.data_ptr(), stream()),
            "ddp_pose_contacts")
    return out


def pairwise_tile(n: int) -> int:
    return 8 if n <= 256 else 4 if n <= 512 else 2


def pose_pairwise_rmsd(pos, perms_t, sel=None, out=None):
    dev = pos.device
    for t, dt, w in ((pos, torch.float32, "pos"), (perms_t, torch.int32, "perms_t")):
        _eval_arg(t, dt, dev, f"pose_pairwise_rmsd {w}")
    if pos.dim() != 3 or pos.shape[2] != 3 or perms_t.dim() != 2:
        raise L.DdpError("pose_pairwise_rmsd: pos [S, rows, 3], perms_t [n, P]")
    S, n, P = pos.shape[0], perms_t.shape[0], perms_t.shape[1]
    if sel is not None:
        _eval_arg(sel, torch.int32, dev, "pose_pairwise_rmsd sel")
        if sel.shape != (n,):
            raise L.DdpError("pose_pairwise_rmsd: sel must have one entry per perms_t row")
    elif n > pos.shape[1]:
        raise L.DdpError("pose_pairwise_rmsd: more perms_t rows than pos rows")
    if out is None:
        out = torch.empty(S, S, dtype=torch.float32, device=dev)
    else:
        _eval_arg(out, torch.float32, dev, "pose_pairwise_rmsd out")
        if out.shape != (S, S):
            raise L.DdpError("pose_pairwise_rmsd: out [S, S]")
    if S == 0:
        return out
    L.check(L.load().ddp_pose_pairwise_rmsd(pos.data_ptr(), S, pos.shape[1] * 3, _p(sel), n, perms_t.data_ptr(), P, out.data_ptr(),
                                            stream()), "ddp_pose_pairwise_rmsd")
    return out


def pose_cluster(dist, order=None, cutoff=2.0):
    dev = dist.device
    _eval_arg(dist, torch.float32, dev, "pose_cluster dist")
    if dist.dim() != 2 or dist.shape[0] != dist.shape[1]:
        raise L.DdpError("pose_cluster: dist [S, S]")
    S = dist.shape[0]
    if order is not None:
        _eval_arg(order, torch.int32, dev, "pose_cluster order")
        if order.shape != (S,):
            raise L.DdpError("pose_cluster: order must have one entry per pose")
    labels, reps, sizes = (torch.empty(S, dtype=torch.int32, device=dev) for _ in range(3))
    count = torch.zeros(1, dtype=torch.int32, device=dev)
    if S == 0:
        return labels, reps, sizes, count
    L.check(L.load().ddp_pose_cluster(dist.data_ptr(), S, _p(order), float(cutoff), labels.data_ptr(), reps.data_ptr(), sizes.data_ptr(),
                                      count.data_ptr(), stream()), "ddp_pose_cluster")
    return labels, reps, sizes, count


def pose_dims(who, pos, rec, per_sample=False):
    dev = pos.device
    _eval_arg(pos, torch.float32, dev, f"{who} pos")
    if pos.dim() != 3 or pos.shape[2] != 3:
        raise L.DdpError(f"{who}: pos [S, n, 3]")
    S, n = pos.shape[0], pos.shape[1]
    if rec.dim() not in ((3,) if per_sample else (2, 3)) or rec.shape[-1] != 3 or (rec.dim() == 3 and rec.shape[0] != S):
        raise L.DdpError(f"{who}: rec [S, m, 3], one receptor per sample" if per_sample else f"{who}: rec [m, 3] or [S, m, 3]")
    m = rec.shape[-2]
    return dev, S, n, m, 3 * m if rec.dim() == 3 else 0


def check_tensors(who, dev, want, optional=(), error=L.DdpError):
    for t, dt, shape, name in want:
        if t is None:
            if optional is None or name in optional:
                continue
            raise error(f"{who} {name}: missing")
        if t.device != dev or t.dtype != dt or not t.is_contiguous():
            raise error(f"{who} {name}: expected a contiguous {dt} tensor on {dev}, got {t.dtype} on {t.device}")
        if shape is not None and tuple(t.shape) != shape:
            raise error(f"{who} {name}: expected {shape}, got {tuple(t.shape)}")


def _pose_args(cls, who, dev, want, optional, config=None, **scalars):
    check_tensors(who, dev, want, optional)
    a = cls(**scalars)
    if config is not None:
        a.form = L.ScoreForm.from_config(config)
    for t, _, _, name in want:
        setattr(a, name, _p(t) or None)
# ... 285 lines not shown
```

diffdock_pocket_amd/score_model.py:

```python
from __future__ import annotations

import math
import os
from typing import Dict, List, Optional

import numpy as np
import torch
from torch import nn

from . import _lib as L
from . import graph as G
from . import launch as K
from . import packing as P
from .synthetic import LIG_FEATURE_DIMS, REC_ATOM_FEATURE_DIMS, REC_RESIDUE_FEATURE_DIMS

ASSETS = os.path.join(os.path.dirname(os.path.abspath(__file__)), "assets")


class GaussianSmearing(nn.Module):

    def __init__(self, start=0.0, stop=5.0, num_gaussians=50):
        super().__init__()
        offset = torch.linspace(start, stop, num_gaussians)
        self.coeff = -0.5 / (offset[1] - offset[0]).item() ** 2
# ... 242 lines not shown
        if path.rows:
            w3 = ea.shape[1] // 3
            segs = [(ea[:, i * w3:], view.eid, ea.shape[1], w3) for i in range(3)]
        else:
            segs = [(ea, view.eid, ea.shape[1], ea.shape[1])]
        task = _make_task(pk, path, x, x.shape[1], view, sh, segs, msg, g=g)
        _launch_convs(self.spec_g if factorized else self.spec, [task], flops_spec=self.spec if factorized else None)
        return msg, csr, path

    def forward(self, node_attr, edge_index, edge_attr, edge_sh, out_nodes=None, reduce="mean", edge_weight=1.0,
                factorized=False):
        if reduce != "mean" or not (isinstance(edge_weight, (int, float)) and edge_weight == 1.0):
            raise NotImplementedError("HIP conv implements reduce='mean', edge_weight=1")
        if edge_index.numel() == 0:
            return torch.tensor(0, dtype=node_attr.dtype, device=node_attr.device)
        msg, csr, _ = self.messages(node_attr, edge_index, edge_attr, edge_sh, out_nodes=out_nodes, factorized=factorized)
        dev = node_attr.device
        n_out = int(out_nodes) if out_nodes is not None else node_attr.shape[0]
        out = torch.zeros((n_out, self.spec.d_out), device=dev, dtype=torch.float32)
        _launch_reduce(out, self.spec.d_out, n_out, self.spec.d_out, [(msg, csr, self.packed(dev))], accumulate=False)
        return out


_require_hip, _stream, _ptr = K.require_hip, K.stream, K.ptr
ConvProfiler, SectionTimer, set_conv_profiler = K.ConvProfiler, K.SectionTimer, K.set_conv_profiler
_EdgeMLPPack, _edge_featurize = K.EdgeMLPPack, K.edge_featurize
_make_task, _launch_convs, _launch_reduce = K.make_task, K.launch_convs, K.launch_reduce


class _EncoderPack:

    def __init__(self, enc, dev):
        tabs = [e.weight.detach().float() for e in enc.atom_embedding_list]
        self.table = torch.cat(tabs, 0).contiguous().to(dev)
        self.feat_off = [0]
        for t in tabs[:-1]:
            self.feat_off.append(self.feat_off[-1] + t.shape[0])
        self.n_cat, self.emb_dim = len(tabs), tabs[0].shape[1]
        self.old = isinstance(enc, OldAtomEncoder)
        if self.old:
            self.has_lm = enc.lm_embedding_type is not None
            self.n_scalar = enc.num_scalar_features
            if self.n_scalar > 0:
                self.w1, self.b1 = enc.linear.weight.detach().float().t().contiguous().to(dev), enc.linear.bias.detach().float().to(dev)
            if self.has_lm:
                lin = enc.lm_embedding_layer
                self.w2, self.b2 = lin.weight.detach().float().t().contiguous().to(dev), lin.bias.detach().float().to(dev)
        else:
            self.has_extra = enc.additional_features_dim > 0
            if self.has_extra:
                lin = enc.additional_features_embedder
                self.w, self.b = lin.weight.detach().float().t().contiguous().to(dev), lin.bias.detach().float().to(dev)


def _node_job(n_rows, out, ncols, w, bias, zero_to=0, cat=None, pack=None, emb_mode=0, dense=(), sigma=None, sig_out=None, add=None):
    j = L.NodeJob()
    j.n_rows, j.out, j.ld_out, j.ncols, j.zero_to = n_rows, out.data_ptr(), out.stride(0), ncols, zero_to
    j.w, j.bias = w.data_ptr(), (bias.data_ptr() if bias is not None else 0)
    if cat is not None and emb_mode:
        j.cat, j.ld_cat, j.n_cat, j.table, j.emb_dim, j.emb_mode = cat.data_ptr(), cat.stride(0), pack.n_cat, pack.table.data_ptr(), pack.emb_dim, emb_mode
        for f, o in enumerate(pack.feat_off):
            j.feat_off[f] = o
    for d, (ten, c0, n) in enumerate(dense):
        j.dense[d], j.ld_dense[d], j.n_dense[d] = ten.data_ptr() + 4 * c0, ten.stride(0), n
    if sigma is not None and sigma[0] == "t":
        _, t, scale, freq, sd = sigma
        j.t, j.t_stride, j.scale, j.freq, j.sd = t.data_ptr(), (t.stride(0) if t.numel() > 1 else 0), scale, freq.data_ptr(), sd
    elif sigma is not None:
        j.sig_emb, j.ld_sig, j.sd = sigma[1].data_ptr(), sigma[1].stride(0), sigma[1].shape[1]
    if sig_out is not None:
        j.sig_out, j.ld_sig_out = sig_out.data_ptr(), sig_out.stride(0)
    if add is not None:
        j.add, j.ld_add = add.data_ptr(), add.stride(0)
    return j


def _launch_node_jobs(jobs):
    lib = L.load()
    for i in range(0, len(jobs), L.DDP_MAX_NODE_JOBS):
        part = jobs[i:i + L.DDP_MAX_NODE_JOBS]
        arr = (L.NodeJob * len(part))(*part)
        L.check(lib.ddp_node_linear(arr, len(part), _stream()), "ddp_node_linear")


class TensorProductScoreModel(nn.Module):
    def __init__(self, t_to_sigma, device, timestep_emb_func, in_lig_edge_features=4, sigma_embed_dim=32, sh_lmax=2,
                 ns=16, nv=4, num_conv_layers=2, lig_max_radius=5, rec_max_radius=30, cross_max_distance=250,
                 center_max_distance=30, distance_embed_dim=32, cross_distance_embed_dim=32, no_torsion=False,
                 scale_by_sigma=True, norm_by_sigma=True, use_second_order_repr=False, batch_norm=True,
                 dynamic_max_cross=False, dropout=0.0, smooth_edges=False, odd_parity=False,
                 separate_noise_schedule=False, lm_embedding_type=False, confidence_mode=False,
                 confidence_dropout=0, confidence_no_batchnorm=False,
                 asyncronous_noise_schedule=False, affinity_prediction=False, parallel=1,
                 parallel_aggregators="mean max min std", num_confidence_outputs=1, fixed_center_conv=False,
                 atom_max_neighbors=None,
                 no_aminoacid_identities=False, flexible_sidechains=False, include_miscellaneous_atoms=False,
                 use_old_atom_encoder=False):
        super().__init__()
        unsupported = {"sh_lmax != 1": sh_lmax != 1, "use_second_order_repr": use_second_order_repr,
                       "odd_parity": odd_parity,
                       "separate_noise_schedule": separate_noise_schedule,
                       "asyncronous_noise_schedule": asyncronous_noise_schedule,
                       "affinity_prediction": affinity_prediction, "parallel > 1": parallel != 1,
                       "include_miscellaneous_atoms": include_miscellaneous_atoms}
        bad = [k for k, v in unsupported.items() if v]
        if bad:
            raise NotImplementedError("MI355X score model: unsupported configuration: " + ", ".join(bad))
        assert (not no_aminoacid_identities) or (lm_embedding_type is None), "no language model emb without identities"
        if num_conv_layers < 1:
            raise NotImplementedError("num_conv_layers >= 1 required")
        self.t_to_sigma = t_to_sigma
        self.device = device
        self.timestep_emb_func = timestep_emb_func
        self.in_lig_edge_features = in_lig_edge_features
        self.sigma_embed_dim = sigma_embed_dim
        self.lig_max_radius, self.rec_max_radius = lig_max_radius, rec_max_radius
        self.cross_max_distance, self.dynamic_max_cross = cross_max_distance, dynamic_max_cross
        self.center_max_distance = center_max_distance
        self.distance_embed_dim, self.cross_distance_embed_dim = distance_embed_dim, cross_distance_embed_dim
        self.ns, self.nv = ns, nv
        self.scale_by_sigma, self.norm_by_sigma = scale_by_sigma, norm_by_sigma
        self.no_torsion = no_torsion
        self.num_conv_layers = num_conv_layers
        self.fixed_center_conv = fixed_center_conv
        self.atom_max_neighbors = atom_max_neighbors
        self.no_aminoacid_identities = no_aminoacid_identities
        self.flexible_sidechains = flexible_sidechains
        self.confidence_mode = bool(confidence_mode)
        self.smooth_edges = bool(smooth_edges)

        enc = OldAtomEncoder if use_old_atom_encoder else AtomEncoder
        sd, dd, cd = sigma_embed_dim, distance_embed_dim, cross_distance_embed_dim
        self.lig_node_embedding = enc(ns, LIG_FEATURE_DIMS, sd)
        self.lig_edge_embedding = _mlp(in_lig_edge_features + sd + dd, ns, ns, dropout)
        self.rec_node_embedding = enc(ns, REC_RESIDUE_FEATURE_DIMS, sd, lm_embedding_type=lm_embedding_type)
        self.rec_edge_embedding = _mlp(sd + dd, ns, ns, dropout)
        self.atom_node_embedding = enc(ns, REC_ATOM_FEATURE_DIMS, sd)
        self.atom_edge_embedding = _mlp(sd + dd, ns, ns, dropout)
        self.lr_edge_embedding = _mlp(sd + cd, ns, ns, dropout)
        self.ar_edge_embedding = _mlp(sd + dd, ns, ns, dropout)
        self.la_edge_embedding = _mlp(sd + cd, ns, ns, dropout)
        self.lig_distance_expansion = GaussianSmearing(0.0, lig_max_radius, dd)
        self.rec_distance_expansion = GaussianSmearing(0.0, rec_max_radius, dd)
        self.cross_distance_expansion = GaussianSmearing(0.0, cross_max_distance, cd)

        def out_blocks(m):
            return [(mul, dim, s) for mul, dim, s in ((m[0], 1, True), (m[1], 3, False), (m[2], 3, False), (m[3], 1, False))
                    if mul > 0]

        convs = []
        self._layer_specs, self._layer_specs_g = [], []
        self.factorize_min_degree = 3.0
        self.prune_last_receptor_layer = True
        self.share_layer0 = True
        self.share_clean_layer1 = True
        self.share_flex_layer0 = True
        self.flex_share_min_work = 2_000_000
        self.plan_min_edges = 0
        self._static_cache = {}
        self.before_layers = None
        self.cache_slot = 0
        self._stage_a_stacks = {}
        self.section_timer = None
        self.check_weight_values = True
        self.range_check_in_forward = True
        self.la_capacity_per_atom = 128
        self.concurrent_small_batches = True
        self.concurrent_max_atoms = 16000
        self.fork_small_means = True
        self.overlap_direct_conv = True
        self.split_rows_launch = True
        self.shape_early_rows = False
        self.split_rows_min_g_bytes = 3.0e9
        self.fork_front = True
        self.fork_lists_flex = True
        self.concurrent_heads = True
        self.stage_a_bf16x3 = False
        self.stage_a_h2 = True
        self._overflow_flag = None
        self.exact_sizes = False
        self.debug_conv_outputs = None
        for i in range(num_conv_layers):
            mi, mo = P.irreps_muls(ns, nv, i), P.irreps_muls(ns, nv, i + 1)
            spec = P.faster_tp_spec(mi, mo, 3 * ns)
            spec_g = P.faster_tp_spec(mi, mo, 3 * ns, factorized=True)
            self._layer_specs.append(spec)
            self._layer_specs_g.append(spec_g)
            for _ in range(9):
                convs.append(TensorProductConvLayer(spec, out_blocks(mo), batch_norm=batch_norm, dropout=dropout,
                                                    spec_g=spec_g))
        self.conv_layers = nn.ModuleList(convs)
        m_final = P.irreps_muls(ns, nv, num_conv_layers)
        self._d_final = P.irreps_dim(m_final)
        self._ldx = (P.irreps_dim(P.irreps_muls(ns, nv, num_conv_layers)) + 3) // 4 * 4

        if self.confidence_mode:
            conf_in = (2 * ns if num_conv_layers >= 3 else ns) * (2 if flexible_sidechains else 1)
            bn = (lambda: nn.Identity()) if confidence_no_batchnorm else (lambda: nn.BatchNorm1d(ns))
            self.confidence_predictor = nn.Sequential(
                nn.Linear(conf_in, ns), bn(), nn.ReLU(), nn.Dropout(confidence_dropout),
                nn.Linear(ns, ns), bn(), nn.ReLU(), nn.Dropout(confidence_dropout),
                nn.Linear(ns, num_confidence_outputs))
        else:
            self.center_distance_expansion = GaussianSmearing(0.0, center_max_distance, dd)
            self.center_edge_embedding = _mlp(dd + sd, ns, ns, dropout)
            self.final_conv = TensorProductConvLayer(P.faster_tp_spec(m_final, (0, 2, 2, 0), 2 * ns),
                                                     [(2, 3, False), (2, 3, False)], batch_norm=batch_norm, dropout=dropout)
            self.tr_final_layer = nn.Sequential(nn.Linear(1 + sd, ns), nn.Dropout(dropout), nn.ReLU(), nn.Linear(ns, 1))
            self.rot_final_layer = nn.Sequential(nn.Linear(1 + sd, ns), nn.Dropout(dropout), nn.ReLU(), nn.Linear(ns, 1))
            tor_blocks = [(ns, 1, False), (ns, 1, True)]
            if not no_torsion:
                self.final_edge_embedding = _mlp(dd, ns, ns, dropout)
                self.tor_bond_conv = TensorProductConvLayer(P.torsion_tp_spec(m_final, ns, 3 * ns), tor_blocks,
                                                            batch_norm=batch_norm, dropout=dropout)
                self.tor_final_layer = nn.Sequential(nn.Linear(2 * ns, ns, bias=False), nn.Tanh(), nn.Dropout(dropout),
                                                     nn.Linear(ns, 1, bias=False))
            if flexible_sidechains:
                self.sidechain_final_edge_embedding = _mlp(dd, ns, ns, dropout)
                self.sc_tor_bond_conv = TensorProductConvLayer(P.torsion_tp_spec(m_final, ns, 3 * ns), tor_blocks,
                                                               batch_norm=batch_norm, dropout=dropout)
                self.sc_tor_final_layer = nn.Sequential(nn.Linear(2 * ns, ns, bias=False), nn.Tanh(), nn.Dropout(dropout),
                                                        nn.Linear(ns, 1, bias=False))
        with np.load(os.path.join(ASSETS, "score_norm_tables.npz")) as z:
            self._so3_table = torch.from_numpy(z["so3_exp_score_norms"]).float()
            self._torus_table = torch.from_numpy(z["torus_score_norm"]).float()
        self._edge_packs: Dict[str, _EdgeMLPPack] = {}
        self.last_stats: Dict[str, float] = {}
        self.rows_mfma16, self.g_planes3, self.direct_rows = rows_defaults()
        self.direct_rows_max_split = int(os.environ.get("DDP_DIRECT_SPLIT", "6"))

    _IGNORED_PREFIXES = ("final_tp_tor.", "final_tp_sc_tor.", "tor_bond_conv.tp.", "sc_tor_bond_conv.tp.")

    def load_state_dict(self, state_dict, strict=True, **kw):
        sd = {k: v for k, v in state_dict.items() if not k.startswith(self._IGNORED_PREFIXES)}
        out = super().load_state_dict(sd, strict=strict, **kw)
        self.invalidate_packed()
        return out

    def _shared_receptor_side(self, B, rec, atom, rpos, apos, lay_r, lay_a, rr, ar, aa, atoms=True):
        out = {3: None, 5: None, 6: None, 8: None}
        if B < 2 or not (lay_r.uniform and lay_a.uniform):
            return out
        nr, na = lay_r.nmax, lay_a.nmax

        def same_rows(t, n):
            v = t.reshape(B, n, -1)
            return bool((v == v[:1]).all())

        def same_edges(ei, n0, n1):
            E = ei.shape[1]
            if E == 0 or E % B:
                return 0
            e = E // B
            off = torch.arange(B, device=ei.device).unsqueeze(1)
            a, b = ei[0].reshape(B, e) - off * n0, ei[1].reshape(B, e) - off * n1
            ok = (a == a[:1]).all() & (b == b[:1]).all() & (a >= 0).all() & (a < n0).all() & (b >= 0).all() & (b < n1).all()
            return e if bool(ok) else 0

        rec_same = same_rows(rec.x, nr) and same_rows(rpos, nr)
        atom_same = atoms is True and same_rows(atom.x, na) and same_rows(apos, na)
        if rec_same:
            e = same_edges(rr, nr, nr)
            out[6] = (nr, e, nr) if e else None
        if atoms == "static" and rec_same and same_rows(atom.x, na):
            e = same_edges(ar, na, nr)
            out["flex"] = (na, e, nr) if e else None
        if atom_same:
            e = same_edges(aa, na, na)
            out[3] = (na, e, na) if e else None
        if rec_same and atom_same:
            e = same_edges(ar, na, nr)
            if e:
                out[5], out[8] = (na, e, nr), (nr, e, na)
        return out

    def _weight_tensors(self):
        ts = self.__dict__.get("_weight_tensors_")
        if ts is None:
            ts = self.__dict__["_weight_tensors_"] = list(self.parameters()) + list(self.buffers())
        return ts

    def _weights_version(self):
        return sum(t._version for t in self._weight_tensors())

    def _weights_fingerprint(self):
        ts = [t.detach() for t in self._weight_tensors() if t.is_floating_point() and t.numel() > 0]
        if not ts:
            return ()
        parts = torch._foreach_norm(ts, 1) + torch._foreach_norm(ts, 2)
        return tuple(torch.stack([p.double() for p in parts]).tolist())

    def _refresh_weight_caches(self):
        wv = self._weights_version()
        fp = self._weights_fingerprint() if self.check_weight_values else self.__dict__.get("_weights_seen_fp")
        if self.__dict__.get("_weights_seen") != wv or self.__dict__.get("_weights_seen_fp") != fp:
            self.invalidate_packed()
            self._weights_seen = wv
            self._weights_seen_fp = fp if self.check_weight_values else self._weights_fingerprint()

    def overflow_flag(self, dev):
        if self._overflow_flag is None:
            self._overflow_flag = torch.zeros(2, dtype=torch.int32).pin_memory()
        return self._overflow_flag

    def check_overflow(self, range_too=True):
        if self._overflow_flag is None:
# ... 283 lines not shown
```

include/ddp_hip.h:

```cpp
#ifndef DDP_HIP_H
#define DDP_HIP_H

#include <stdint.h>

#ifdef __cplusplus
extern "C" {
#endif

#define DDP_ABI_VERSION 17
#define DDP_EINVAL (-1)
#define DDP_ELIMIT (-2)

#define DDP_MAX_TASKS 9
#define DDP_MAX_BLOCKS 4
#define DDP_MAX_SEGS 3
#define DDP_MAX_NS 64
#define DDP_EDGE_TILE 64

enum ddp_feat_kind {
  DDP_F_SCALAR_S0 = 0,
  DDP_F_DOT = 1,
  DDP_F_SCALAR_S1 = 2,
  DDP_F_VEC_S0 = 3,
  DDP_F_CROSS = 4
// ... 191 lines not shown
  float* out;
} ddp_tor_args_t;
int ddp_tor_head(const ddp_tor_args_t* args, void* stream);

#define DDP_MAX_GEMM_BATCH 16
#define DDP_G_LD(hid, gcols) ((((((hid) + 3) / 4) * 4 + 1) * (gcols) + 31) / 32 * 32)
int ddp_stage_a(const float* x, int ldx, int nrows, const int32_t* rows, const int32_t* nrows_dev, int out_rows, const int32_t* offs,
                int nbatch, const float* w, const void* w_bf16x3, int k, int ncols, float* out, int ldo, void* stream);

int ddp_stage_a_h2(const float* x, int ldx, int nrows, const int32_t* rows, const int32_t* nrows_dev, int out_rows, const int32_t* offs,
                   int nbatch, const float* w, const void* w_h2, int k, int ncols, float* out, int ldo, int32_t* range_flag, void* stream);
int ddp_stage_a_gh(const float* x, int ldx, int nrows, const int32_t* rows, const int32_t* nrows_dev, int out_rows, const int32_t* offs,
                   int nbatch, const float* w, const void* w_h2, int k, int ncols, float* out, int ldo, int32_t* range_flag,
                   const int32_t* dest, void* stream);

int ddp_stage_a_gh3(const float* x, int ldx, int nrows, const int32_t* rows, const int32_t* nrows_dev, int out_rows, const int32_t* offs,
                    int nbatch, const float* w, const void* w_h2, int k, int ncols, float* out, int ldo, int32_t* range_flag,
                    const int32_t* dest, void* stream);

#define DDP_GH_SX 2

int ddp_set_occupancy_shaping(int rows_min_lds_bytes, int stage_a_lds_pad_bytes);

extern int ddp_sa_drainwave;

extern int ddp_conv_deal;
int ddp_conv_deal_tile(int id, int total, int c);

int ddp_pose_update(const float* pos_in, int n_samples, int n_atoms, const float* tr, const float* rot, const float* tor,
                    int n_tor, const int32_t* bonds, const uint8_t* mask_rotate, float* pos_out, void* stream);

int ddp_sidechain_update(const float* pos_in, int n_samples, int n_atoms, const float* angles, int n_bonds,
                         const int32_t* edge_idx, const int32_t* subcomponents, const int32_t* mapping, float* pos_out,
                         void* stream);

typedef struct {
  const float* score[4];
  const float* z[4];
  float* out[4];
  int32_t n[4];
} ddp_sde_args_t;
int ddp_sde_update(const float* coef, const ddp_sde_args_t* args, void* stream);

#define DDP_RADIUS_DROP_SELF 1
#define DDP_RADIUS_NEAREST 2
int ddp_radius_count(const float* x, const int32_t* x_ptr, const float* y, const int32_t* y_batch, int ny, float r,
                     int max_neighbors, int flags, int32_t* counts, void* stream);
int ddp_radius_fill(const float* x, const int32_t* x_ptr, const float* y, const int32_t* y_batch, int ny, float r,
                    int max_neighbors, int flags, const int32_t* offsets, int32_t* out_query, int32_t* out_x, void* stream);
int ddp_knn(const float* x, const int32_t* x_ptr, const int32_t* batch, int n, int k, int32_t* out_neighbors, void* stream);

int ddp_group_by_key(const int32_t* key, int n_items, int n_keys, const int32_t* pay0, const int32_t* pay1, const int32_t* pay2,
                     int32_t* rowptr, int32_t* perm, int32_t* out_key, int32_t* out0, int32_t* out1, int32_t* out2,
                     int32_t* scratch, void* stream);

#define DDP_MAX_LIST_JOBS 12

typedef struct {
  int32_t n;
  const int32_t* n_dev;
  const int32_t* flag;
  const int32_t* val;
  const int32_t* rowptr;
  int32_t base;
  int32_t* excl;
  int32_t* excl2;
  int32_t* list;
  int32_t* total;
} ddp_scan_job_t;
int ddp_scan_jobs(const ddp_scan_job_t* jobs, int njobs, void* stream);

typedef struct {
  const int32_t* idx;
  int32_t n;
  const int32_t* n_dev;
  int32_t* mask;
} ddp_mark_job_t;
int ddp_mark_jobs(const ddp_mark_job_t* jobs, int njobs, void* stream);

typedef struct {
  int32_t n_rows;
  const int32_t* keep;
  const int32_t* old_rowptr;
  const int32_t* new_rowptr;
  const int32_t* in[3];
  int32_t* out[3];
} ddp_rowcopy_job_t;
int ddp_rowcopy_jobs(const ddp_rowcopy_job_t* jobs, int njobs, void* stream);

typedef struct {
  int32_t n;
  const int32_t* n_dev;
  const int32_t* mask_a;
  const int32_t* idx_a;
  const int32_t* mask_b;
  const int32_t* idx_b;
  int32_t* out_idx;
  const int32_t* pay[4];
  int32_t pay_add[4];
  int32_t* out[4];
  int32_t* total;
  int32_t* block_count;
  int32_t* block_off;
} ddp_select_job_t;
int ddp_select_jobs(const ddp_select_job_t* jobs, int njobs, void* stream);

int ddp_gather_rows(const float* x, int ldx, const int32_t* idx, int n, const int32_t* n_dev, float* out, int ldo, int ncols,
                    void* stream);

int ddp_clean_pair_maps(const int32_t* touched, const int32_t* recv, const int32_t* src, const int32_t* rowptr, int n_edges, int e0,
                        int n_graphs, int n0, int32_t* rowmap, int32_t* rows_v, void* stream);

int ddp_flex_mark(const float* pos, const int32_t* flag, int n_b_per_graph, const int32_t* a, const int32_t* b, int n_edges, int e0,
                  int n_a_per_graph, int a_too, int ref_list, int32_t* mark, void* stream);
int ddp_fallback_rowmap(const int32_t* mark, const int32_t* recv, const int32_t* old_rowptr, const int32_t* new_rowptr, int n_edges,
                        int n_recv_per_graph, int32_t* rowmap, void* stream);

typedef struct {
  const float* x;
  const int32_t* x_ptr;
  const float* y;
  const int32_t* y_batch;
  int32_t ny;
  float r;
  int32_t max_neighbors;
  int32_t flags;
  const float* graph_div;
  int32_t* counts;
  int32_t* offsets;
  int32_t base;
  int32_t* total;
  int32_t* out_query;
  int32_t* out_x;
  int32_t capacity;
  int32_t* overflow;
} ddp_radius_job_t;
int ddp_radius_search_jobs(const ddp_radius_job_t* jobs, int njobs, void* stream);

typedef struct {
  const int32_t* key;
  int32_t n_items;
  const int32_t* n_items_dev;
  int32_t n_keys;
  const int32_t* pay[3];
  int32_t* rowptr;
  int32_t* perm;
  int32_t* out_key;
  int32_t* out[3];
  const int32_t* key_map;
  int32_t* scratch;
} ddp_group_job_t;
int ddp_group_by_key_jobs(const ddp_group_job_t* jobs, int njobs, void* stream);

#define DDP_MAX_NODE_JOBS 8
#define DDP_MAX_NODE_CAT 16
typedef struct {
  int32_t n_rows;
  const int32_t* cat;
  int32_t ld_cat, n_cat;
  const float* table;
  int32_t feat_off[DDP_MAX_NODE_CAT];
  int32_t emb_dim, emb_mode;
  const float* dense[2];
  int32_t ld_dense[2], n_dense[2];
  const float* t;
  int32_t t_stride;
  float scale;
  const float* freq;
  const float* sig_emb;
  int32_t ld_sig, sd;
  float* sig_out;
  int32_t ld_sig_out;
  const float* w;
  const float* bias;
  float* out;
  int32_t ld_out, ncols, zero_to;
  const float* add;
  int32_t ld_add;
} ddp_node_job_t;
int ddp_node_linear(const ddp_node_job_t* jobs, int njobs, void* stream);

#define DDP_EVAL_MAX_ATOMS 1024

int ddp_pose_rmsd(const float* pred, int n_samples, int pred_stride, const int32_t* sel, int n, const float* ref, int n_ref,
                  const int32_t* perms, int n_perms, float* rmsd, int32_t* best, void* stream);

int ddp_pose_contacts(const float* lig, int n_samples, int n, const float* lig_radii, const float* rec, int m, int rec_stride,
                      const float* rec_radii, float overlap, const float* ref_centroid, float* out, void* stream);

#define DDP_PAIRWISE_MAX_SAMPLES 32768

int ddp_pose_pairwise_rmsd(const float* pos, int n_samples, int pos_stride, const int32_t* sel, int n, const int32_t* perms, int n_perms,
                           float* dist, void* stream);

int ddp_pose_cluster(const float* dist, int n_samples, const int32_t* order, float cutoff, int32_t* labels, int32_t* reps, int32_t* sizes,
                     int32_t* n_clusters, void* stream);

int ddp_traj_record(const float* lig_pos, int n, int n_lig, float* lig_traj, const float* atom_pos, int n_atoms, const int32_t* moving,
                    int n_moving, float* atom_traj, int n_slots, const float* slot, void* stream);

typedef struct {
  const float* pos;
  int32_t n, n_lig, n_tor;
  const int32_t* dihedrals;
  const float* score[3];
  float* upd[3];
  const float* gdt;
  float weight, w_rep, w_rot, w_tor;
  int32_t svgd_only;
  double* tau;
  float* tr_diff;
  float* rot_diff;
  float* tor_diff;
  double* dist;
} ddp_svgd_args_t;
int ddp_svgd_tau(const ddp_svgd_args_t* args, void* stream);
int ddp_svgd_pairs(const ddp_svgd_args_t* args, void* stream);
int ddp_svgd_rows(const ddp_svgd_args_t* args, void* stream);

typedef struct {
  int32_t n_samples, n, m, rec_stride, n_tor;
  float* pos;
  const float* anchor;
  const float* lig_radii;
  const float* rec;
  const float* rec_radii;
  const uint8_t* self_pairs;
  double overlap, restraint;
  double* energy;
  double* grad;
  const int32_t* bonds;
  const uint8_t* mask_rotate;
  double* step;
  float* tr;
  float* rot;
  float* tor;
  const float* trial;
  const double* trial_energy;
  const double* trial_grad;
  int32_t* accepted;
  double grow, shrink, step_max;
} ddp_refine_args_t;
int ddp_refine_energy(const ddp_refine_args_t* args, void* stream);
int ddp_refine_direction(const ddp_refine_args_t* args, void* stream);
int ddp_refine_accept(const ddp_refine_args_t* args, void* stream);

typedef struct {
  double cutoff;
  double gauss_offset, gauss_width;
  double hydrophobic_good, hydrophobic_bad;
  double hbond_good, hbond_bad;
  double w_gauss, w_repulsion, w_hydrophobic, w_hbond;
} ddp_score_form_t;

typedef struct {
  int32_t n_samples, n, m, rec_stride;
  const float* pos;
  const float* lig_radii;
  const uint8_t* lig_flags;
  const float* rec;
  const float* rec_radii;
  const uint8_t* rec_flags;
  const uint8_t* self_pairs;
  ddp_score_form_t form;
  double tor_divisor;
  double* energy;
  double* grad;
} ddp_score_args_t;
int ddp_pose_score(const ddp_score_args_t* args, void* stream);

typedef struct {
  int32_t n_samples, n, m, rec_stride, n_res, reserved;
  const float* pos;
  const float* lig_radii;
  const uint8_t* lig_flags;
  const float* rec;
  const float* rec_radii;
  const uint8_t* rec_flags;
  const int32_t* res_ptr;
  ddp_score_form_t form;
  double contact_distance;
  double* profile;
  uint8_t* bits;
} ddp_profile_args_t;
int ddp_pose_profile(const ddp_profile_args_t* args, void* stream);

#define DDP_MINIMIZE_MAX_ATOMS 512
#define DDP_MINIMIZE_MAX_TORSIONS 4096
typedef struct {
  int32_t n_samples, n, m, rec_stride, n_tor, iterations;
  float* pos;
  const float* anchor;
  const float* lig_radii;
  const uint8_t* lig_flags;
  const float* rec;
  const float* rec_radii;
  const uint8_t* rec_flags;
  const uint8_t* self_pairs;
  const int32_t* bonds;
  const uint8_t* mask_rotate;
  ddp_score_form_t form;
  double restraint, grow, shrink, step_max;
  double* step;
  int32_t* accepted;
  double* energy_in;
  double* energy_out;
// ... 177 lines not shown
```

Measured before the change: 178.5.

## Fuse per-graph radius searches and CSR grouping into one front-lists kernel

Adds a per-graph kernel that builds ligand-ligand, ligand-receptor, ligand-atom and torsion neighbour masks in LDS with wave ballots. It then emits the edge lists, receiver CSR rowptrs, column (source-ordered) views and near-row lists directly. This replaces the chain of radius search, scan and group-by-key launches when the graph sizes fit the fixed limits. The aim is to cut launch count and global-memory passes in the per-step graph construction. The cost is a large LDS footprint per block, a count pass plus a fill pass, and a fallback path kept for oversized graphs.

```diff
diff --git a/diffdock_pocket_amd/_lib.py b/diffdock_pocket_amd/_lib.py
--- a/diffdock_pocket_amd/_lib.py
+++ b/diffdock_pocket_amd/_lib.py
@@ -21,7 +21,7 @@
 DDP_PAIRWISE_MAX_SAMPLES, DDP_CLUSTER_MAX_SAMPLES = 32768, 1024
 EXPORTS = ["ddp_conv_messages", "ddp_conv_rows", "ddp_stage_a_gh", "ddp_stage_a_gh3", "ddp_segment_reduce", "ddp_edge_featurize", "ddp_edge_featurize_jobs", "ddp_torsion_sh", "ddp_stage_a", "ddp_stage_a_h2",
            "ddp_pose_update", "ddp_sidechain_update", "ddp_sde_update", "ddp_radius_count", "ddp_radius_fill", "ddp_knn", "ddp_group_by_key", "ddp_node_linear", "ddp_scan_jobs", "ddp_mark_jobs", "ddp_rowcopy_jobs", "ddp_select_jobs",
-           "ddp_gather_rows", "ddp_clean_pair_maps", "ddp_flex_mark", "ddp_fallback_rowmap", "ddp_step_prologue", "ddp_trrot_head", "ddp_tor_head", "ddp_radius_search_jobs", "ddp_group_by_key_jobs", "ddp_set_occupancy_shaping", "ddp_pose_rmsd", "ddp_pose_contacts", "ddp_pose_pairwise_rmsd", "ddp_pose_cluster", "ddp_traj_record", "ddp_svgd_tau", "ddp_svgd_pairs", "ddp_svgd_rows", "ddp_refine_energy", "ddp_refine_direction", "ddp_refine_accept", "ddp_clash_guidance", "ddp_score_guidance", "ddp_score_guidance_flex", "ddp_pose_score", "ddp_pose_profile", "ddp_pose_minimize", "ddp_pose_minimize_flex", "ddp_pose_search", "ddp_pose_search_select", "ddp_pose_search_flex", "ddp_pocket_occupancy", "ddp_pocket_buriedness", "ddp_pocket_label", "ddp_conv_deal_tile", "ddp_abi_version", "ddp_last_error", "ddp_source_hash"]
+           "ddp_gather_rows", "ddp_clean_pair_maps", "ddp_flex_mark", "ddp_fallback_rowmap", "ddp_step_prologue", "ddp_trrot_head", "ddp_tor_head", "ddp_radius_search_jobs", "ddp_group_by_key_jobs", "ddp_front_lists", "ddp_set_occupancy_shaping", "ddp_pose_rmsd", "ddp_pose_contacts", "ddp_pose_pairwise_rmsd", "ddp_pose_cluster", "ddp_traj_record", "ddp_svgd_tau", "ddp_svgd_pairs", "ddp_svgd_rows", "ddp_refine_energy", "ddp_refine_direction", "ddp_refine_accept", "ddp_clash_guidance", "ddp_score_guidance", "ddp_score_guidance_flex", "ddp_pose_score", "ddp_pose_profile", "ddp_pose_minimize", "ddp_pose_minimize_flex", "ddp_pose_search", "ddp_pose_search_select", "ddp_pose_search_flex", "ddp_pocket_occupancy", "ddp_pocket_buriedness", "ddp_pocket_label", "ddp_conv_deal_tile", "ddp_abi_version", "ddp_last_error", "ddp_source_hash"]
 
 
 class Seg(C.Structure):
@@ -195,6 +195,32 @@
 class GroupJob(C.Structure):
     _fields_ = [("key", _P), ("n_items", _I), ("n_items_dev", _P), ("n_keys", _I), ("pay", _P * 3), ("rowptr", _P), ("perm", _P),
                 ("out_key", _P), ("out", _P * 3), ("key_map", _P), ("scratch", _P)]
+
+
+DDP_FRONT_MAX_LIG, DDP_FRONT_MAX_REC, DDP_FRONT_MAX_ATOM, DDP_FRONT_MAX_BONDS = 64, 256, 2048, 256
+
+
+class FrontView(C.Structure):
+    _fields_ = [("rowptr", _P), ("perm", _P), ("key", _P), ("out0", _P), ("out1", _P)]
+
+
+class FrontLists(C.Structure):
+    _fields_ = [("n_graphs", _I), ("n_lig", _I), ("n_rec", _I), ("n_atom", _I), ("n_tor", _I),
+                ("max_lig", _I), ("max_rec", _I), ("max_atom", _I), ("max_tor", _I), ("max_bonds", _I),
+                ("lig_pos", _P), ("rec_pos", _P), ("atom_pos", _P), ("tor_pos", _P),
+                ("lig_ptr", _P), ("rec_ptr", _P), ("atom_ptr", _P), ("tor_ptr", _P),
+                ("r_lig", C.c_float), ("r_cross", C.c_float), ("cross_div", _P),
+                ("ll_neighbors", _I), ("tor_neighbors", _I), ("cross_neighbors", _I), ("la_neighbors", _I),
+                ("radius_flags", _I), ("e_bond", _I),
+                ("ll0", _P), ("ll1", _P), ("cap_ll", _I), ("cnt_ll", _P),
+                ("lr0", _P), ("lr1", _P), ("cap_lr", _I), ("cnt_lr", _P),
+                ("la0", _P), ("la1", _P), ("cap_la", _I), ("cnt_la", _P), ("overflow", _P),
+                ("tor_q", _P), ("tor_x", _P), ("cap_tor", _I), ("cnt_tor", _P),
+                ("touched", _P), ("near_rows", _P), ("cnt_near", _P),
+                ("rp_lr", _P), ("rp_la", _P), ("rp_tor", _P),
+                ("c_ll", FrontView), ("c_la", FrontView), ("c_lr", FrontView),
+                ("so_ll", FrontView), ("so_la", FrontView), ("so_lr", FrontView),
+                ("scratch", _P)]
 
 
 
@@ -315,6 +341,8 @@
                       ("ddp_select_jobs", SelectJob), ("ddp_radius_search_jobs", RadiusJob), ("ddp_group_by_key_jobs", GroupJob)):
         getattr(lib, name).argtypes = [C.POINTER(job), C.c_int, C.c_void_p]
         getattr(lib, name).restype = C.c_int
+    lib.ddp_front_lists.argtypes = [C.POINTER(FrontLists), C.POINTER(C.c_int32), C.c_void_p]
+    lib.ddp_front_lists.restype = C.c_int
     lib.ddp_sde_update.argtypes = [C.c_void_p, C.POINTER(SdeArgs), C.c_void_p]
     lib.ddp_sde_update.restype = C.c_int
     lib.ddp_gather_rows.argtypes = [C.c_void_p, C.c_int, C.c_void_p, C.c_int, C.c_void_p, C.c_void_p, C.c_int, C.c_int, C.c_void_p]
diff --git a/diffdock_pocket_amd/build.py b/diffdock_pocket_amd/build.py
--- a/diffdock_pocket_amd/build.py
+++ b/diffdock_pocket_amd/build.py
@@ -7,9 +7,9 @@
 
 HERE = os.path.dirname(os.path.abspath(__file__))
 ROOT = os.path.dirname(HERE)
-SOURCES = ["ddp_conv.hip", "ddp_conv_rows.hip", "ddp_conv_rows16.hip", "ddp_misc.hip", "ddp_gemm.hip", "ddp_pose.hip", "ddp_graph.hip", "ddp_views.hip", "ddp_lists.hip", "ddp_node.hip", "ddp_heads.hip",
+SOURCES = ["ddp_conv.hip", "ddp_conv_rows.hip", "ddp_conv_rows16.hip", "ddp_misc.hip", "ddp_gemm.hip", "ddp_pose.hip", "ddp_graph.hip", "ddp_views.hip", "ddp_lists.hip", "ddp_front_lists.hip", "ddp_node.hip", "ddp_heads.hip",
            "ddp_eval.hip", "ddp_traj.hip", "ddp_svgd.hip", "ddp_refine.hip", "ddp_guidance.hip", "ddp_score_guidance.hip", "ddp_score_guidance_flex.hip", "ddp_score.hip", "ddp_profile.hip", "ddp_minimize.hip", "ddp_minimize_flex.hip", "ddp_search.hip", "ddp_search_flex.hip", "ddp_pockets.hip", "ddp_capi.hip"]
-HEADERS = [os.path.join(HERE, "csrc", "ddp_internal.h"), os.path.join(HERE, "csrc", "ddp_conv_diag.h"), os.path.join(HERE, "csrc", "ddp_conv_common.h"), os.path.join(HERE, "csrc", "ddp_conv_deal.h"), os.path.join(HERE, "csrc", "ddp_conv_rows_common.h"), os.path.join(HERE, "csrc", "ddp_horn.h"), os.path.join(HERE, "csrc", "ddp_pockets_uf.h"), os.path.join(HERE, "csrc", "ddp_score_pair.h"), os.path.join(HERE, "csrc", "ddp_pose_descent.h"), os.path.join(HERE, "csrc", "ddp_minimize_loop.h"), os.path.join(HERE, "csrc", "ddp_minimize_flex_loop.h"), os.path.join(HERE, "csrc", "ddp_clash_energy.h"),
+HEADERS = [os.path.join(HERE, "csrc", "ddp_internal.h"), os.path.join(HERE, "csrc", "ddp_conv_diag.h"), os.path.join(HERE, "csrc", "ddp_conv_common.h"), os.path.join(HERE, "csrc", "ddp_conv_deal.h"), os.path.join(HERE, "csrc", "ddp_conv_rows_common.h"), os.path.join(HERE, "csrc", "ddp_horn.h"), os.path.join(HERE, "csrc", "ddp_pockets_uf.h"), os.path.join(HERE, "csrc", "ddp_score_pair.h"), os.path.join(HERE, "csrc", "ddp_pose_descent.h"), os.path.join(HERE, "csrc", "ddp_minimize_loop.h"), os.path.join(HERE, "csrc", "ddp_minimize_flex_loop.h"), os.path.join(HERE, "csrc", "ddp_clash_energy.h"), os.path.join(HERE, "csrc", "ddp_radius_math.h"),
            os.path.join(ROOT, "include", "ddp_hip.h")]
 OUT = os.path.join(HERE, "libddp_hip.so")
 OBJ_DIR = os.path.join(HERE, "csrc", ".obj")
diff --git a/diffdock_pocket_amd/csrc/ddp_front_lists.hip b/diffdock_pocket_amd/csrc/ddp_front_lists.hip
--- /dev/null
+++ b/diffdock_pocket_amd/csrc/ddp_front_lists.hip
@@ -0,0 +1,485 @@
+#include <hip/hip_runtime.h>
+#include <stdint.h>
+
+#include "ddp_hip.h"
+#include "ddp_internal.h"
+#include "ddp_radius_math.h"
+
+#define FL_THREADS 1024
+#define FL_WAVES (FL_THREADS / 64)
+#define FL_NL DDP_FRONT_MAX_LIG
+#define FL_WR (DDP_FRONT_MAX_REC / 64)
+#define FL_WA (DDP_FRONT_MAX_ATOM / 64)
+#define FL_NB DDP_FRONT_MAX_BONDS
+#define FL_PART_LISTS 0
+#define FL_PART_LA 1
+#define FL_PART_C_LA 2
+#define FL_PART_C_LR 3
+#define FL_PART_LL 4
+#define FL_PARTS 5
+static_assert(FL_NL == 64, "a ligand row of the masks is one 64-bit word");
+
+typedef unsigned long long u64;
+
+struct FrontLds {
+  float lp[3 * FL_NL], lps[3 * FL_NL], tp[3 * FL_NL];
+  u64 mll[FL_NL], mtor[FL_NL], mlr[FL_NL * FL_WR], mla[FL_NL * FL_WA];
+  unsigned short plr[FL_NL * FL_WR], pla[FL_NL * FL_WA];
+  int off[4][FL_NL + 1];
+  int wsum[FL_WAVES];
+  int tot[8], base[8];
+  int nbond;
+  int bl[FL_NB], bk0[FL_NB], bk1[FL_NB], posb[FL_NB];
+  int nb0[FL_NL], nb1[FL_NL], rs0[FL_NL], rs1[FL_NL];
+  int posr[FL_NL * FL_NL];
+};
+
+__device__ __forceinline__ u64 bits_below(int b) { return (1ull << b) - 1ull; }
+
+__device__ __forceinline__ u64 first_bits(u64 m, int cap) {
+  while (__popcll(m) > cap) m &= ~(1ull << (63 - __clzll((long long)m)));
+  return m;
+}
+
+__device__ __forceinline__ int wave_incl_scan(int v, int lane) {
+#pragma unroll
+  for (int d = 1; d < 64; d <<= 1) {
+    const int t = __shfl_up(v, d);
+    if (lane >= d) v += t;
+  }
+  return v;
+}
+
+__device__ int block_excl_scan(int v, int* wsum, int& total) {
+  const int lane = (int)threadIdx.x & 63, wid = (int)threadIdx.x >> 6;
+  const int incl = wave_incl_scan(v, lane);
+  if (lane == 63) wsum[wid] = incl;
+  __syncthreads();
+  int pre = 0, tot = 0;
+#pragma unroll
+  for (int w = 0; w < FL_WAVES; ++w) {
+    const int t = wsum[w];
+    tot += t;
+    if (w < wid) pre += t;
+  }
+  __syncthreads();
+  total = tot;
+  return pre + incl - v;
+}
+
+__device__ __forceinline__ int clamp_count(int n, int cap) { return n < cap ? (n < 0 ? 0 : n) : cap; }
+
+template <int W, bool NEAR>
+__device__ void column_view(const u64* mask, const unsigned short* pre, const int* off, int nq, int ncols, int base, int n, int x0,
+                            int q0, int n_nodes, bool last, const ddp_front_view_t& c, int32_t* so_perm, int* wsum,
+                            int32_t* near_rows, int near_base) {
+  const int tid = (int)threadIdx.x;
+  const int rbase = base < n ? base : n;
+  int carry = 0, ncarry = 0;
+  for (int j0 = 0; j0 < ncols; j0 += FL_THREADS) {
+    const int j = j0 + tid, w = j >> 6, b = j & 63;
+    int cc = 0, tc = 0;
+    if (j < ncols)
+      for (int q = 0; q < nq; ++q) {
+        const u64 m = mask[q * W + w];
+        if ((m >> b) & 1ull) {
+          ++tc;
+          cc += (base + off[q] + (int)pre[q * W + w] + __popcll(m & bits_below(b))) < n ? 1 : 0;
+        }
+      }
+    int total;
+    const int ex = block_excl_scan(cc, wsum, total) + carry;
+    if (j < ncols) {
+      c.rowptr[x0 + j] = rbase + ex;
+      int k = 0;
+      for (int q = 0; q < nq && k < cc; ++q) {
+        const u64 m = mask[q * W + w];
+        if ((m >> b) & 1ull) {
+          const int orig = base + off[q] + (int)pre[q * W + w] + __popcll(m & bits_below(b));
+          const int p = rbase + ex + k;
+          c.perm[p] = orig;
+          c.key[p] = x0 + j;
+          c.out0[p] = q0 + q;
+          so_perm[orig] = p;
+          ++k;
+        }
+      }
+    }
+    carry += total;
+    if (NEAR) {
+      int ntot;
+      const int ex2 = block_excl_scan(tc != 0 ? 1 : 0, wsum, ntot) + ncarry;
+      if (j < ncols && tc != 0) near_rows[near_base + ex2] = x0 + j;
+      ncarry += ntot;
+    }
+  }
+  if (last)
+    for (int i = x0 + ncols + tid; i <= n_nodes; i += FL_THREADS) c.rowptr[i] = n;
+}
+
+template <bool FILL>
+__global__ __launch_bounds__(FL_THREADS) void ddp_front_lists_kernel(const ddp_front_lists_t A) {
+  __shared__ FrontLds S;
+  const int g = (int)blockIdx.x, tid = (int)threadIdx.x, lane = tid & 63, wid = tid >> 6;
+  const int part = FILL ? (int)blockIdx.y : -1;
+  const bool need_ll = !FILL || part == FL_PART_LISTS || part == FL_PART_LL, need_tor = !FILL || part == FL_PART_LISTS;
+  const bool need_lr = !FILL || part == FL_PART_LISTS || part == FL_PART_C_LR, need_la = !FILL || part == FL_PART_LA || part == FL_PART_C_LA;
+  const int l0 = A.lig_ptr[g], nl = A.lig_ptr[g + 1] - l0;
+  const int r0 = A.rec_ptr[g], nr = A.rec_ptr[g + 1] - r0;
+  const int a0 = A.atom_ptr[g], na = A.atom_ptr[g + 1] - a0;
+  const bool tor = A.tor_pos != nullptr && A.n_tor > 0;
+  const int t0 = tor ? A.tor_ptr[g] : 0, nt = tor ? A.tor_ptr[g + 1] - t0 : 0;
+  if (nl < 0 || nl > FL_NL || nt < 0 || nt > FL_NL || nr < 0 || nr > DDP_FRONT_MAX_REC || na < 0 || na > DDP_FRONT_MAX_ATOM) {
+    if (!FILL && tid < 8) A.scratch[8 * g + tid] = 0;
+    return;
+  }
+  const bool scaled = A.cross_div != nullptr;
+  const float div = scaled ? A.cross_div[g] : 1.f;
+  const float r2l = A.r_lig * A.r_lig, r2c = A.r_cross * A.r_cross;
+
+  for (int i = tid; i < nl; i += FL_THREADS) {
+    load_pt(A.lig_pos, (size_t)(l0 + i), false, 1.f, &S.lp[3 * i]);
+    load_pt(A.lig_pos, (size_t)(l0 + i), scaled, div, &S.lps[3 * i]);
+  }
+  for (int i = tid; i < nt; i += FL_THREADS) load_pt(A.tor_pos, (size_t)(t0 + i), false, 1.f, &S.tp[3 * i]);
+  if (tid < 8) S.tot[tid] = S.base[tid] = 0;
+  if (tid < FL_NL) S.nb0[tid] = S.nb1[tid] = 0;
+  if (tid == 0) S.nbond = 0;
+  __syncthreads();
+
+  const int Wr = (nr + 63) >> 6, Wa = (na + 63) >> 6;
+  for (int task = wid; task < 2 + Wr + Wa; task += FL_WAVES) {
+    float xj[3] = {0.f, 0.f, 0.f};
+    if (task == 0 ? !need_ll : task == 1 ? !need_tor : task < 2 + Wr ? !need_lr : !need_la) continue;
+    if (task < 2) {
+      const bool valid = lane < nl;
+      if (valid) { xj[0] = S.lp[3 * lane]; xj[1] = S.lp[3 * lane + 1]; xj[2] = S.lp[3 * lane + 2]; }
+      if (task == 0) {
+        for (int q = 0; q < nl; ++q) {
+          const u64 mm = __ballot(valid && sqdist(&S.lp[3 * q], xj) < r2l);
+          if (lane == 0) S.mll[q] = first_bits(mm, A.ll_neighbors) & ~(1ull << q);
+        }
+      } else {
+        for (int q = 0; q < nt; ++q) {
+          const u64 mm = __ballot(valid && sqdist(&S.tp[3 * q], xj) < r2l);
+          if (lane == 0) S.mtor[q] = first_bits(mm, A.tor_neighbors);
+        }
+      }
+    } else if (task < 2 + Wr) {
+      const int w = task - 2, j = 64 * w + lane;
+      const bool valid = j < nr;
+      if (valid) load_pt(A.rec_pos, (size_t)(r0 + j), scaled, div, xj);
+      for (int q = 0; q < nl; ++q) {
+        const u64 mm = __ballot(valid && sqdist(&S.lps[3 * q], xj) < r2c);
+        if (lane == 0) S.mlr[q * FL_WR + w] = mm;
+      }
+    } else {
+      const int w = task - 2 - Wr, j = 64 * w + lane;
+      const bool valid = j < na;
+      if (valid) load_pt(A.atom_pos, (size_t)(a0 + j), false, 1.f, xj);
+      int c = 0;
+      for (int q = 0; q < nl; ++q) {
+        const bool m = valid && sqdist(&S.lp[3 * q], xj) < r2l;
+        const u64 mm = __ballot(m);
+        c += m ? 1 : 0;
+        if (lane == 0) S.mla[q * FL_WA + w] = mm;
+      }
+      if (!FILL) {
+        if (valid) A.touched[a0 + j] = c;
+        const u64 nz = __ballot(c != 0);
+        if (lane == 0) atomicAdd(&S.tot[4], __popcll(nz));
+      }
+    }
+  }
+  for (int i = tid; i < (need_ll && part != FL_PART_LISTS ? A.e_bond : 0); i += FL_THREADS) {
+    const int k = A.ll0[i] - l0;
+    if ((unsigned)k < (unsigned)nl) {
+      const int slot = atomicAdd(&S.nbond, 1);
+      if (FILL && slot < FL_NB) S.bl[slot] = i;
+    }
+  }
+  __syncthreads();
+
+  if (tid < 256) {
+    const int q = lane;
+    int c = 0;
+    if (wid == 0) {
+      if (q < nl) c = __popcll(S.mll[q]);
+    } else if (wid == 1) {
+      if (q < nl)
+        for (int w = 0; w < Wr; ++w) { S.plr[q * FL_WR + w] = (unsigned short)c; c += __popcll(S.mlr[q * FL_WR + w]); }
+    } else if (wid == 2) {
+      if (q < nl)
+        for (int w = 0; w < Wa; ++w) { S.pla[q * FL_WA + w] = (unsigned short)c; c += __popcll(S.mla[q * FL_WA + w]); }
+    } else if (q < nt) {
+      c = __popcll(S.mtor[q]);
+    }
+    const int incl = wave_incl_scan(c, lane);
+    S.off[wid][q] = incl - c;
+    if (lane == 63) S.off[wid][FL_NL] = incl;
+  }
+  __syncthreads();
+
+  if (!FILL) {
+    if (tid < 8) {
+      int v = 0;
+      if (tid < 4) v = S.off[tid][FL_NL];
+      else if (tid == 4) v = S.tot[4];
+      else if (tid == 5) v = S.nbond;
+      A.scratch[8 * g + tid] = v;
+    }
+    return;
+  }
+
+  for (int idx = tid; idx < 8 * A.n_graphs; idx += FL_THREADS) {
+    const int v = A.scratch[idx], s = idx & 7;
+    if (v != 0) {
+      atomicAdd(&S.tot[s], v);
+      if ((idx >> 3) < g) atomicAdd(&S.base[s], v);
+    }
+  }
+  __syncthreads();
+  const int Eb = A.e_bond;
+  const int n_ll = clamp_count(Eb + S.tot[0], A.cap_ll), n_lr = clamp_count(S.tot[1], A.cap_lr);
+  const int n_la = clamp_count(S.tot[2], A.cap_la), n_tor = clamp_count(S.tot[3], A.cap_tor);
+  const int b_ll = Eb + S.base[0], b_lr = S.base[1], b_la = S.base[2], b_tor = S.base[3], b_near = S.base[4], b_bond = S.base[5];
+  const bool last = g == A.n_graphs - 1;
+  if (g == 0 && tid == 0 && part == FL_PART_LISTS) {
+    *A.cnt_ll = Eb + S.tot[0];
+    *A.cnt_lr = S.tot[1];
+    *A.cnt_la = S.tot[2];
+    *A.cnt_near = S.tot[4];
+    if (tor) *A.cnt_tor = S.tot[3];
+  }
+
+  for (int row = wid; row < nl; row += FL_WAVES) {
+    const int q = l0 + row;
+    if (part == FL_PART_LISTS) {
+      const u64 m = S.mll[row];
+      if ((m >> lane) & 1ull) {
+        const int o = b_ll + S.off[0][row] + __popcll(m & bits_below(lane));
+        if (o < A.cap_ll) {
+          A.ll1[o] = q;
+          A.ll0[o] = l0 + lane;
+        }
+      }
+    }
+    for (int w = 0; w < (part == FL_PART_LISTS ? Wr : 0); ++w) {
+      const u64 m = S.mlr[row * FL_WR + w];
+      if ((m >> lane) & 1ull) {
+        const int o = b_lr + S.off[1][row] + (int)S.plr[row * FL_WR + w] + __popcll(m & bits_below(lane));
+        if (o < A.cap_lr) {
+          const int x = r0 + 64 * w + lane;
+          A.lr0[o] = q;
+          A.lr1[o] = x;
+          A.so_lr.key[o] = q;
+          A.so_lr.out0[o] = x;
+          A.so_lr.out1[o] = o;
+        }
+      }
+    }
+    for (int w = 0; w < (part == FL_PART_LA ? Wa : 0); ++w) {
+      const u64 m = S.mla[row * FL_WA + w];
+      if ((m >> lane) & 1ull) {
+        const int o = b_la + S.off[2][row] + (int)S.pla[row * FL_WA + w] + __popcll(m & bits_below(lane));
+        if (o < A.cap_la) {
+          const int x = a0 + 64 * w + lane;
+          A.la0[o] = q;
+          A.la1[o] = x;
+          A.so_la.key[o] = q;
+          A.so_la.out0[o] = x;
+          A.so_la.out1[o] = o;
+        } else if (A.overflow) {
+          *A.overflow = 1;
+        }
+      }
+    }
+  }
+  for (int row = wid; row < (part == FL_PART_LISTS ? nt : 0); row += FL_WAVES) {
+    const u64 m = S.mtor[row];
+    if ((m >> lane) & 1ull) {
+      const int o = b_tor + S.off[3][row] + __popcll(m & bits_below(lane));
+      if (o < A.cap_tor) {
+        A.tor_q[o] = t0 + row;
+        A.tor_x[o] = l0 + lane;
+      }
+    }
+  }
+  if (part == FL_PART_LISTS) {
+    if (tid < nl) {
+      const int vr = min(b_lr + S.off[1][tid], n_lr);
+      A.rp_lr[l0 + tid] = vr;
+      if (A.so_lr.rowptr) A.so_lr.rowptr[l0 + tid] = vr;
+    }
+    if (tid < nt) A.rp_tor[t0 + tid] = min(b_tor + S.off[3][tid], n_tor);
+    if (last) {
+      for (int i = l0 + nl + tid; i <= A.n_lig; i += FL_THREADS) {
+        A.rp_lr[i] = n_lr;
+        if (A.so_lr.rowptr) A.so_lr.rowptr[i] = n_lr;
+      }
+      if (tor)
+        for (int i = t0 + nt + tid; i <= A.n_tor; i += FL_THREADS) A.rp_tor[i] = n_tor;
+    }
+    return;
+  }
+  if (part == FL_PART_LA) {
+    if (tid < nl) {
+      const int va = min(b_la + S.off[2][tid], n_la);
+      A.rp_la[l0 + tid] = va;
+      if (A.so_la.rowptr) A.so_la.rowptr[l0 + tid] = va;
+    }
+    if (last)
+      for (int i = l0 + nl + tid; i <= A.n_lig; i += FL_THREADS) {
+        A.rp_la[i] = n_la;
+        if (A.so_la.rowptr) A.so_la.rowptr[i] = n_la;
+      }
+    return;
+  }
+
+  if (part == FL_PART_C_LA) {
+    column_view<FL_WA, true>(S.mla, S.pla, S.off[2], nl, na, b_la, n_la, a0, l0, A.n_atom, last, A.c_la, A.so_la.perm, S.wsum, A.near_rows,
+                             b_near);
+    return;
+  }
+  if (part == FL_PART_C_LR) {
+    column_view<FL_WR, false>(S.mlr, S.plr, S.off[1], nl, nr, b_lr, n_lr, r0, l0, A.n_rec, last, A.c_lr, A.so_lr.perm, S.wsum, nullptr, 0);
+    return;
+  }
+
+  const int nb = S.nbond < FL_NB ? S.nbond : FL_NB;
+  int myb = 0, rank = 0;
+  if (tid < nb) {
+    myb = S.bl[tid];
+    for (int a = 0; a < nb; ++a) rank += S.bl[a] < myb ? 1 : 0;
+  }
+  __syncthreads();
+  if (tid < nb) S.bl[rank] = myb;
+  __syncthreads();
+  if (tid < nb) {
+    const int i = S.bl[tid];
+    const int k0 = A.ll0[i] - l0;
+    int k1 = A.ll1[i] - l0;
+    if ((unsigned)k1 >= (unsigned)nl) k1 = k0;
+    S.bk0[tid] = k0;
+    S.bk1[tid] = k1;
+    atomicAdd(&S.nb0[k0], 1);
+    atomicAdd(&S.nb1[k1], 1);
+  }
+  __syncthreads();
+  const int rb = b_bond + max(min(b_ll, n_ll) - Eb, 0);
+  if (wid == 0) {
+    const int k = lane;
+    int cc = 0;
+    if (k < nl)
+      for (int q = 0; q < nl; ++q) {
+        const u64 m = S.mll[q];
+        if ((m >> k) & 1ull) cc += (b_ll + S.off[0][q] + __popcll(m & bits_below(k))) < n_ll ? 1 : 0;
+      }
+    const int len = k < nl ? S.nb0[k] + cc : 0;
+    const int ex = wave_incl_scan(len, lane) - len;
+    S.rs0[k] = ex;
+    if (k < nl) {
+      A.c_ll.rowptr[l0 + k] = rb + ex;
+      int kk = 0;
+      for (int q = 0; q < nl && kk < cc; ++q) {
+        const u64 m = S.mll[q];
+        if ((m >> k) & 1ull) {
+          const int p = rb + ex + S.nb0[k] + kk;
+          A.c_ll.perm[p] = b_ll + S.off[0][q] + __popcll(m & bits_below(k));
+          A.c_ll.key[p] = l0 + k;
+          A.c_ll.out0[p] = l0 + q;
+          S.posr[q * FL_NL + k] = p;
+          ++kk;
+        }
+      }
+    }
+  } else if (wid == 1) {
+    const int q = lane;
+    int len = 0;
+    if (q < nl) len = S.nb1[q] + max(min(n_ll - (b_ll + S.off[0][q]), __popcll(S.mll[q])), 0);
+    const int ex = wave_incl_scan(len, lane) - len;
+    S.rs1[q] = ex;
+    if (q < nl && A.so_ll.rowptr) A.so_ll.rowptr[l0 + q] = rb + ex;
+  }
+  if (last)
+    for (int i = l0 + nl + tid; i <= A.n_lig; i += FL_THREADS) {
+      A.c_ll.rowptr[i] = n_ll;
+      if (A.so_ll.rowptr) A.so_ll.rowptr[i] = n_ll;
+    }
+  __syncthreads();
+  if (tid < nb) {
+    const int k = S.bk0[tid];
+    int rnk = 0;
+    for (int a = 0; a < tid; ++a) rnk += S.bk0[a] == k ? 1 : 0;
+    const int p = rb + S.rs0[k] + rnk;
+    A.c_ll.perm[p] = S.bl[tid];
+    A.c_ll.key[p] = l0 + k;
+    A.c_ll.out0[p] = l0 + S.bk1[tid];
+    S.posb[tid] = p;
+  }
+  __syncthreads();
+  for (int idx = tid; idx < nl * FL_NL + nb; idx += FL_THREADS) {
+    int q, mypos, x, orig;
+    if (idx < nl * FL_NL) {
+      q = idx >> 6;
+      const int j = idx & 63;
+      const u64 m = S.mll[q];
+      if (!((m >> j) & 1ull)) continue;
+      orig = b_ll + S.off[0][q] + __popcll(m & bits_below(j));
+      if (orig >= n_ll) continue;
+      mypos = S.posr[q * FL_NL + j];
+      x = l0 + j;
+    } else {
+      const int a = idx - nl * FL_NL;
+      q = S.bk1[a];
+      mypos = S.posb[a];
+      x = l0 + S.bk0[a];
+      orig = S.bl[a];
+    }
+    int rnk = 0;
+    const u64 m = S.mll[q];
+    for (u64 t = m; t != 0; t &= t - 1) {
+      const int j2 = __ffsll((long long)t) - 1;
+      if ((b_ll + S.off[0][q] + __popcll(m & bits_below(j2))) < n_ll) rnk += S.posr[q * FL_NL + j2] < mypos ? 1 : 0;
+    }
+    for (int a = 0; a < nb; ++a) rnk += (S.bk1[a] == q && S.posb[a] < mypos) ? 1 : 0;
+    const int p = rb + S.rs1[q] + rnk;
+    A.so_ll.perm[p] = mypos;
+    A.so_ll.key[p] = l0 + q;
+    A.so_ll.out0[p] = x;
+    A.so_ll.out1[p] = orig;
+  }
+}
+
+extern "C" int ddp_front_lists(const ddp_front_lists_t* a, int32_t* taken, void* stream) {
+  if (!a || !taken) return ddp_fail(DDP_EINVAL, "ddp_front_lists: null argument");
+  *taken = 0;
+  const ddp_front_lists_t& A = *a;
+  if (A.n_graphs < 1 || A.n_lig < 0 || A.n_rec < 0 || A.n_atom < 0 || A.n_tor < 0 || A.e_bond < 0)
+    return ddp_fail(DDP_EINVAL, "ddp_front_lists: n_graphs / node totals / e_bond");
+  if (!(A.r_lig > 0.f) || !(A.r_cross > 0.f) || A.ll_neighbors < 1 || A.tor_neighbors < 1 || A.cross_neighbors < 1 || A.la_neighbors < 1)
+    return ddp_fail(DDP_EINVAL, "ddp_front_lists: radius / max_neighbors");
+  if (A.cap_ll < A.e_bond || A.cap_lr < 0 || A.cap_la < 0 || A.cap_tor < 0) return ddp_fail(DDP_EINVAL, "ddp_front_lists: capacities");
+  const bool tor = A.tor_pos != nullptr && A.n_tor > 0;
+  if (!A.lig_pos || !A.rec_pos || !A.atom_pos || !A.lig_ptr || !A.rec_ptr || !A.atom_ptr || !A.scratch || !A.ll0 || !A.ll1 || !A.cnt_ll ||
+      !A.lr0 || !A.lr1 || !A.cnt_lr || !A.la0 || !A.la1 || !A.cnt_la || !A.touched || !A.near_rows || !A.cnt_near || !A.rp_lr || !A.rp_la ||
+      (tor && (!A.tor_ptr || !A.tor_q || !A.tor_x || !A.cnt_tor || !A.rp_tor)))
+    return ddp_fail(DDP_EINVAL, "ddp_front_lists: null argument");
+  const ddp_front_view_t* views[6] = {&A.c_ll, &A.c_la, &A.c_lr, &A.so_ll, &A.so_la, &A.so_lr};
+  for (int i = 0; i < 6; ++i) {
+    const ddp_front_view_t& v = *views[i];
+    if (!v.perm || !v.key || !v.out0 || (i < 3 && !v.rowptr) || (i >= 3 && !v.out1)) return ddp_fail(DDP_EINVAL, "ddp_front_lists: null view array");
+  }
+  if ((A.radius_flags & DDP_RADIUS_NEAREST) != 0) return 0;
+  if (A.max_lig > DDP_FRONT_MAX_LIG || A.max_tor > DDP_FRONT_MAX_LIG || A.max_rec > DDP_FRONT_MAX_REC || A.max_atom > DDP_FRONT_MAX_ATOM ||
+      A.max_bonds > DDP_FRONT_MAX_BONDS)
+    return 0;
+  if (A.cross_neighbors < A.max_rec || A.la_neighbors < A.max_atom) return 0;
+  hipStream_t st = (hipStream_t)stream;
+  hipLaunchKernelGGL((ddp_front_lists_kernel<false>), dim3(A.n_graphs), dim3(FL_THREADS), 0, st, A);
+  hipLaunchKernelGGL((ddp_front_lists_kernel<true>), dim3(A.n_graphs, FL_PARTS), dim3(FL_THREADS), 0, st, A);
+  const hipError_t err = hipGetLastError();
+  if (err != hipSuccess) return ddp_fail_hip(err, "ddp_front_lists launch");
+  *taken = 1;
+  return 0;
+}
diff --git a/diffdock_pocket_amd/csrc/ddp_graph.hip b/diffdock_pocket_amd/csrc/ddp_graph.hip
--- a/diffdock_pocket_amd/csrc/ddp_graph.hip
+++ b/diffdock_pocket_amd/csrc/ddp_graph.hip
@@ -3,32 +3,9 @@
 
 #include "ddp_hip.h"
 #include "ddp_internal.h"
+#include "ddp_radius_math.h"
 
 #define DDP_KNN_MAX 32
-
-__device__ __forceinline__ float sqdist(const float* __restrict__ a, const float* __restrict__ b) {
-#pragma clang fp contract(off)
-  const float dx = a[0] - b[0], dy = a[1] - b[1], dz = a[2] - b[2];
-  const float xx = dx * dx, yy = dy * dy, zz = dz * dz;
-  return (xx + yy) + zz;
-}
-
-__device__ __forceinline__ void load_pt(const float* __restrict__ p, size_t j, bool scaled, float div, float out[3]) {
-  out[0] = p[3 * j];
-  out[1] = p[3 * j + 1];
-  out[2] = p[3 * j + 2];
-  if (scaled) {
-    out[0] = __fdiv_rn(out[0], div);
-    out[1] = __fdiv_rn(out[1], div);
-    out[2] = __fdiv_rn(out[2], div);
-  }
-}
-
-__device__ __forceinline__ float sqdist_to(const float* __restrict__ yq, const float* __restrict__ x, size_t j, bool scaled, float div) {
-  float xj[3];
-  load_pt(x, j, scaled, div, xj);
-  return sqdist(yq, xj);
-}
 
 #define DDP_CUT_LIST 64
 __device__ float radius_cut(const float* __restrict__ x, int j0, int j1, const float* __restrict__ yq, float r2, int cap, bool scaled,
diff --git a/diffdock_pocket_amd/csrc/ddp_radius_math.h b/diffdock_pocket_amd/csrc/ddp_radius_math.h
--- /dev/null
+++ b/diffdock_pocket_amd/csrc/ddp_radius_math.h
@@ -0,0 +1,27 @@
+#pragma once
+#include <hip/hip_runtime.h>
+#include <stddef.h>
+
+__device__ __forceinline__ float sqdist(const float* __restrict__ a, const float* __restrict__ b) {
+#pragma clang fp contract(off)
+  const float dx = a[0] - b[0], dy = a[1] - b[1], dz = a[2] - b[2];
+  const float xx = dx * dx, yy = dy * dy, zz = dz * dz;
+  return (xx + yy) + zz;
+}
+
+__device__ __forceinline__ void load_pt(const float* __restrict__ p, size_t j, bool scaled, float div, float out[3]) {
+  out[0] = p[3 * j];
+  out[1] = p[3 * j + 1];
+  out[2] = p[3 * j + 2];
+  if (scaled) {
+    out[0] = __fdiv_rn(out[0], div);
+    out[1] = __fdiv_rn(out[1], div);
+    out[2] = __fdiv_rn(out[2], div);
+  }
+}
+
+__device__ __forceinline__ float sqdist_to(const float* __restrict__ yq, const float* __restrict__ x, size_t j, bool scaled, float div) {
+  float xj[3];
+  load_pt(x, j, scaled, div, xj);
+  return sqdist(yq, xj);
+}
diff --git a/diffdock_pocket_amd/engine.py b/diffdock_pocket_amd/engine.py
--- a/diffdock_pocket_amd/engine.py
+++ b/diffdock_pocket_amd/engine.py
@@ -50,6 +50,14 @@
 
     def __len__(self):
         return len(self._resolve())
+
+
+def front_lists_fusable(m, S):
+    if not m.fused_front_lists or S.num_flex != 0 or S.sc is not None:
+        return False
+    big = lambda lay: max(lay.counts_host) if lay.counts_host else 0
+    return (big(S.lay_l) <= L.DDP_FRONT_MAX_LIG and big(S.lay_r) <= L.DDP_FRONT_MAX_REC and big(S.lay_a) <= L.DDP_FRONT_MAX_ATOM
+            and S.max_bonds <= L.DDP_FRONT_MAX_BONDS and (S.tor is None or big(S.tor.lay) <= L.DDP_FRONT_MAX_LIG))
 
 
 def _i32(t):
@@ -166,6 +174,14 @@
         S.bond_ei = bond_ei
         S.bond32 = m._cached("bond32", (bond_ei,), lambda: (_i32(bond_ei[0]), _i32(bond_ei[1])))
         S.E_bond = int(bond_ei.shape[1])
+
+        def bond_stats():
+            if S.E_bond == 0:
+                return 0
+            gb = lbatch[bond_ei[0].long()]
+            same = bool((gb == lbatch[bond_ei[1].long()]).all())
+            return int(torch.bincount(gb, minlength=B).max()) if same else 1 << 30
+        S.max_bonds = m._cached("max_bonds", (bond_ei, lig.batch), bond_stats)
         rr, ar = data["receptor", "receptor"].edge_index, data["atom", "receptor"].edge_index
         S.rr, S.ar = rr, ar
         S.num_flex = 0
@@ -273,6 +289,65 @@
         L.check(L.load().ddp_step_prologue(C.byref(a), K.stream()), "ddp_step_prologue")
         F.keep_pro = (keep, a)
 
+    def _search_chain(self, S, F, dev, ll0, ll1, lr0, lr1, la0, la1, cut, b32_l, b32_a):
+        m = self.m
+        Nl, Nr, Na, Eb = S.Nl, S.Nr, S.Na, S.E_bond
+        lpos, rpos, apos, cnt = F.lpos, F.rpos, F.apos, F.cnt
+        ptr_l, ptr_r, ptr_a = S.lay_l._ptr32, S.lay_r._ptr32, S.lay_a._ptr32
+        i32e = lambda n: torch.empty(n, dtype=torch.int32, device=dev)
+        jobs = [K.radius_job(lpos, ptr_l, lpos, b32_l, m.lig_max_radius, 33, _DROP_SELF, i32e(Nl), i32e(Nl + 1), base=Eb,
+                             total=cnt["ll"], out_query=ll1, out_x=ll0, capacity=S.cap_ll)]
+        if m.dynamic_max_cross:
+            jobs.append(K.radius_job(rpos, ptr_r, lpos, b32_l, 1.0, 10000, 0, i32e(Nl), i32e(Nl + 1), total=cnt["lr"],
+                                     out_query=lr0, out_x=lr1, capacity=S.cap_lr, graph_div=cut))
+        else:
+            jobs.append(K.radius_job(rpos, ptr_r, lpos, b32_l, m.cross_max_distance, 10000, 0, i32e(Nl), i32e(Nl + 1), total=cnt["lr"],
+                                     out_query=lr0, out_x=lr1, capacity=S.cap_lr))
+        jobs.append(K.radius_job(apos, ptr_a, lpos, b32_l, m.lig_max_radius, 10000, 0, i32e(Nl), i32e(Nl + 1), total=cnt["la"],
+                                 out_query=la0, out_x=la1, capacity=S.cap_la, overflow=m.overflow_flag(dev)))
+        jobs.append(K.radius_job(lpos, ptr_l, apos, b32_a, m.lig_max_radius, 10000, 0, F.touched))
+        for name, st, pos, ptr_x in (("tor", S.tor, lpos, ptr_l), ("sc", S.sc, apos, ptr_a)):
+            if st is None:
+                continue
+            h = getattr(F, name)
+            h.q, h.x = i32e(st.cap), i32e(st.cap)
+            jobs.append(K.radius_job(pos, ptr_x, h.bond_pos, G._batch32(st.lay, st.T), m.lig_max_radius, 32, 0, i32e(st.T),
+                                     i32e(st.T + 1), total=cnt[name], out_query=h.q, out_x=h.x, capacity=st.cap))
+            setattr(F, name, h)
+        K.radius_search_jobs(jobs)
+        F.keep += [jobs, cut]
+        K.scan_jobs([K.scan_job(Na, flag=F.touched, lst=F.near_rows, total=cnt["near"])])
+
+    def _fused_lists(self, S, F, dev, ll0, ll1, lr0, lr1, la0, la1, cut):
+        m = self.m
+        Nl, Nr, Na, cnt = S.Nl, S.Nr, S.Na, F.cnt
+        i32e = lambda n: torch.empty(n, dtype=torch.int32, device=dev)
+
+        def view(n_keys, cap, o1=False):
+            return SimpleNamespace(rp=i32e(n_keys + 1), perm=i32e(cap), key=i32e(cap), o0=i32e(cap), o1=i32e(cap) if o1 else None)
+        V = SimpleNamespace(c_ll=view(Nl, S.cap_ll), c_la=view(Na, S.cap_la), c_lr=view(Nr, S.cap_lr), so_ll=view(Nl, S.cap_ll, True),
+                            so_la=view(Nl, S.cap_la, True), so_lr=view(Nl, S.cap_lr, True), rp_lr=i32e(Nl + 1), rp_la=i32e(Nl + 1))
+        h, tor, T, max_t = F.tor, None, 0, 0
+        if h is not None:
+            st = h.st
+            T, max_t = st.T, max(st.lay.counts_host)
+            h.q, h.x, h.rp = i32e(st.cap), i32e(st.cap), i32e(T + 1)
+            tor = (h.q, h.x, st.cap, cnt["tor"], h.rp)
+        scratch = i32e(8 * S.B)
+        maxes = (max(S.lay_l.counts_host), max(S.lay_r.counts_host), max(S.lay_a.counts_host), max_t, S.max_bonds)
+        taken = K.front_lists(
+            n_graphs=S.B, sizes=(Nl, Nr, Na, T), maxes=maxes, pos=(F.lpos, F.rpos, F.apos, h.bond_pos if h is not None else None),
+            ptrs=(S.lay_l._ptr32, S.lay_r._ptr32, S.lay_a._ptr32, h.st.lay._ptr32 if h is not None else None),
+            r_lig=m.lig_max_radius, r_cross=1.0 if cut is not None else m.cross_max_distance, cross_div=cut, neighbors=(33, 32, 10000, 10000),
+            e_bond=S.E_bond, ll=(ll0, ll1, S.cap_ll, cnt["ll"]), lr=(lr0, lr1, S.cap_lr, cnt["lr"]),
+            la=(la0, la1, S.cap_la, cnt["la"], m.overflow_flag(dev)), tor=tor, touched=F.touched, near_rows=F.near_rows,
+            cnt_near=cnt["near"], rp_lr=V.rp_lr, rp_la=V.rp_la,
+            views={k: getattr(V, k) for k in ("c_ll", "c_la", "c_lr", "so_ll", "so_la", "so_lr")}, scratch=scratch)
+        if not taken:
+            return None
+        F.keep += [V, scratch, cut]
+        return V
+
     def _front(self, data, S, lig, rec, atom, dev, mark, ff=None):
         m = self.m
         ns, B = m.ns, S.B
@@ -309,32 +384,13 @@
         F.aa = aa
         S.stats["E_aa"] = int(aa.shape[1])
         lr0, lr1, la0, la1 = i32e(S.cap_lr), i32e(S.cap_lr), i32e(S.cap_la), i32e(S.cap_la)
-        jobs = [K.radius_job(lpos, ptr_l, lpos, b32_l, m.lig_max_radius, 33, _DROP_SELF, i32e(Nl), i32e(Nl + 1), base=Eb,
-                             total=cnt["ll"], out_query=ll1, out_x=ll0, capacity=S.cap_ll)]
-        cut = None
-        if m.dynamic_max_cross:
-            cut = F.cut
-            jobs.append(K.radius_job(rpos, ptr_r, lpos, b32_l, 1.0, 10000, 0, i32e(Nl), i32e(Nl + 1), total=cnt["lr"],
-                                     out_query=lr0, out_x=lr1, capacity=S.cap_lr, graph_div=cut))
-        else:
-            jobs.append(K.radius_job(rpos, ptr_r, lpos, b32_l, m.cross_max_distance, 10000, 0, i32e(Nl), i32e(Nl + 1), total=cnt["lr"],
-                                     out_query=lr0, out_x=lr1, capacity=S.cap_lr))
-        jobs.append(K.radius_job(apos, ptr_a, lpos, b32_l, m.lig_max_radius, 10000, 0, i32e(Nl), i32e(Nl + 1), total=cnt["la"],
-                                 out_query=la0, out_x=la1, capacity=S.cap_la, overflow=m.overflow_flag(dev)))
-        F.touched = i32e(Na)
-        jobs.append(K.radius_job(lpos, ptr_l, apos, b32_a, m.lig_max_radius, 10000, 0, F.touched))
-        for name, st, pos, ptr_x in (("tor", S.tor, lpos, ptr_l), ("sc", S.sc, apos, ptr_a)):
-            if st is None:
-                continue
-            h = getattr(F, name)
-            h.q, h.x = i32e(st.cap), i32e(st.cap)
-            jobs.append(K.radius_job(pos, ptr_x, h.bond_pos, G._batch32(st.lay, st.T), m.lig_max_radius, 32, 0, i32e(st.T),
-                                     i32e(st.T + 1), total=cnt[name], out_query=h.q, out_x=h.x, capacity=st.cap))
-            setattr(F, name, h)
-        K.radius_search_jobs(jobs)
-        F.keep = [jobs, cut]
-        F.near_rows = i32e(Na)
-        K.scan_jobs([K.scan_job(Na, flag=F.touched, lst=F.near_rows, total=cnt["near"])])
+        F.touched, F.near_rows = i32e(Na), i32e(Na)
+        cut = F.cut if m.dynamic_max_cross else None
+        F.keep = []
+        fv = self._fused_lists(S, F, dev, ll0, ll1, lr0, lr1, la0, la1, cut) if front_lists_fusable(m, S) else None
+        S.stats["front_fused"] = int(fv is not None)
+        if fv is None:
+            self._search_chain(S, F, dev, ll0, ll1, lr0, lr1, la0, la1, cut, b32_l, b32_a)
         mark("searches")
 
         shared0 = {}
@@ -403,21 +459,25 @@
         c[5] = static_csr("c_ar", 5, S.ar, S.ar[0], S.ar[1], Na)
         c[6] = static_csr("c_rr", 6, rr, rr[0], rr[1], Nr)
         c[8] = static_csr("c_ra", 8, S.ar, S.ar[1], S.ar[0], Nr)
-        v = SimpleNamespace(rp=i32e(Nl + 1), perm=i32e(S.cap_ll), key=i32e(S.cap_ll), o0=i32e(S.cap_ll))
-        g1.append(K.group_job(ll0, S.cap_ll, Nl, [ll1], v.rp, v.perm, v.key, [v.o0], i32e(Nl + S.cap_ll), n_dev=cnt["ll"]))
+        v = fv.c_ll if fv is not None else SimpleNamespace(rp=i32e(Nl + 1), perm=i32e(S.cap_ll), key=i32e(S.cap_ll), o0=i32e(S.cap_ll))
+        if fv is None:
+            g1.append(K.group_job(ll0, S.cap_ll, Nl, [ll1], v.rp, v.perm, v.key, [v.o0], i32e(Nl + S.cap_ll), n_dev=cnt["ll"]))
         c[0] = EdgeView(S.cap_ll, v.key, v.o0, v.perm, rowptr=v.rp, cnt=cnt["ll"])
         for k, q0, x1, cap, name in ((1, lr0, lr1, S.cap_lr, "lr"), (2, la0, la1, S.cap_la, "la")):
-            rp = i32e(Nl + 1)
-            g1.append(K.group_job(q0, cap, Nl, [], rp, scratch=i32e(Nl), n_dev=cnt[name]))
+            rp = getattr(fv, "rp_" + name) if fv is not None else i32e(Nl + 1)
+            if fv is None:
+                g1.append(K.group_job(q0, cap, Nl, [], rp, scratch=i32e(Nl), n_dev=cnt[name]))
             c[k] = EdgeView(cap, q0, x1, G.iota32(cap, dev), rowptr=rp, cnt=cnt[name])
         for k, key, pay, cap, n_keys, name in ((4, la1, la0, S.cap_la, Na, "la"), (7, lr1, lr0, S.cap_lr, Nr, "lr")):
-            v = SimpleNamespace(rp=i32e(n_keys + 1), perm=i32e(cap), key=i32e(cap), o0=i32e(cap))
-            g1.append(K.group_job(key, cap, n_keys, [pay], v.rp, v.perm, v.key, [v.o0], i32e(n_keys + cap), n_dev=cnt[name]))
+            v = getattr(fv, "c_" + name) if fv is not None else SimpleNamespace(rp=i32e(n_keys + 1), perm=i32e(cap), key=i32e(cap), o0=i32e(cap))
+            if fv is None:
+                g1.append(K.group_job(key, cap, n_keys, [pay], v.rp, v.perm, v.key, [v.o0], i32e(n_keys + cap), n_dev=cnt[name]))
             c[k] = EdgeView(cap, v.key, v.o0, v.perm, rowptr=v.rp, cnt=cnt[name])
         for h, name in ((F.tor, "tor"), (F.sc, "sc")):
             if h is not None:
-                h.rp = i32e(h.st.T + 1)
-                g1.append(K.group_job(h.q, h.st.cap, h.st.T, [], h.rp, scratch=i32e(h.st.T), n_dev=cnt[name]))
+                if fv is None:
+                    h.rp = i32e(h.st.T + 1)
+                    g1.append(K.group_job(h.q, h.st.cap, h.st.T, [], h.rp, scratch=i32e(h.st.T), n_dev=cnt[name]))
                 h.csr = EdgeView(h.st.cap, h.q, h.x, G.iota32(h.st.cap, dev), rowptr=h.rp, cnt=cnt[name])
         K.group_jobs(g1)
         F.keep.append(g1)
@@ -440,9 +500,12 @@
                 g2.append(K.group_job(c[3].src, E3, Na, [c[3].recv, c[3].eid], v.rp, v.perm, v.key, [v.o0, v.o1], i32e(Na + E3)))
                 so[3] = G.SourceOrder(E3, v.o0, v.key, v.o1, v.perm)
             for k, cap, name in ((0, S.cap_ll, "ll"), (4, S.cap_la, "la"), (7, S.cap_lr, "lr")):
-                v = SimpleNamespace(rp=i32e(Nl + 1), perm=i32e(cap), key=i32e(cap), o0=i32e(cap), o1=i32e(cap))
-                g2.append(K.group_job(c[k].src, cap, Nl, [c[k].recv, c[k].eid], v.rp, v.perm, v.key, [v.o0, v.o1], i32e(Nl + cap),
-                                      n_dev=cnt[name]))
+                if fv is not None:
+                    v = getattr(fv, "so_" + name)
+                else:
+                    v = SimpleNamespace(rp=i32e(Nl + 1), perm=i32e(cap), key=i32e(cap), o0=i32e(cap), o1=i32e(cap))
+                    g2.append(K.group_job(c[k].src, cap, Nl, [c[k].recv, c[k].eid], v.rp, v.perm, v.key, [v.o0, v.o1], i32e(Nl + cap),
+                                          n_dev=cnt[name]))
                 so[k] = EdgeView(cap, v.o0, v.key, v.o1, pos=v.perm, cnt=cnt[name])
             K.group_jobs(g2)
             F.keep.append(g2)
diff --git a/diffdock_pocket_amd/launch.py b/diffdock_pocket_amd/launch.py
--- a/diffdock_pocket_amd/launch.py
+++ b/diffdock_pocket_amd/launch.py
@@ -494,6 +494,32 @@
 
 def group_jobs(jobs: Sequence[L.GroupJob]):
     _run_jobs("ddp_group_by_key_jobs", L.GroupJob, list(jobs), "ddp_group_by_key_jobs")
+
+
+def front_lists(*, n_graphs, sizes, maxes, pos, ptrs, r_lig, r_cross, cross_div, neighbors, e_bond, ll, lr, la, tor, touched, near_rows,
+                cnt_near, rp_lr, rp_la, views, scratch, flags=0) -> bool:
+    a = L.FrontLists()
+    a.n_graphs = n_graphs
+    a.n_lig, a.n_rec, a.n_atom, a.n_tor = sizes
+    a.max_lig, a.max_rec, a.max_atom, a.max_tor, a.max_bonds = maxes
+    a.lig_pos, a.rec_pos, a.atom_pos, a.tor_pos = (_p(t) for t in pos)
+    a.lig_ptr, a.rec_ptr, a.atom_ptr, a.tor_ptr = (_p(t) for t in ptrs)
+    a.r_lig, a.r_cross, a.cross_div = float(r_lig), float(r_cross), _p(cross_div)
+    a.ll_neighbors, a.tor_neighbors, a.cross_neighbors, a.la_neighbors = neighbors
+    a.radius_flags, a.e_bond = int(flags), int(e_bond)
+    a.ll0, a.ll1, a.cap_ll, a.cnt_ll = _p(ll[0]), _p(ll[1]), int(ll[2]), _p(ll[3])
+    a.lr0, a.lr1, a.cap_lr, a.cnt_lr = _p(lr[0]), _p(lr[1]), int(lr[2]), _p(lr[3])
+    a.la0, a.la1, a.cap_la, a.cnt_la, a.overflow = _p(la[0]), _p(la[1]), int(la[2]), _p(la[3]), _p(la[4])
+    if tor is not None:
+        a.tor_q, a.tor_x, a.cap_tor, a.cnt_tor, a.rp_tor = _p(tor[0]), _p(tor[1]), int(tor[2]), _p(tor[3]), _p(tor[4])
+    a.touched, a.near_rows, a.cnt_near, a.rp_lr, a.rp_la = _p(touched), _p(near_rows), _p(cnt_near), _p(rp_lr), _p(rp_la)
+    for name, v in views.items():
+        f = getattr(a, name)
+        f.rowptr, f.perm, f.key, f.out0, f.out1 = _p(v.rp), _p(v.perm), _p(v.key), _p(v.o0), _p(getattr(v, "o1", None))
+    a.scratch = _p(scratch)
+    taken = C.c_int32(0)
+    L.check(L.load().ddp_front_lists(C.byref(a), C.byref(taken), stream()), "ddp_front_lists")
+    return bool(taken.value)
 
 
 def gather_rows(x, idx, n, out, ncols, n_dev=None):
diff --git a/diffdock_pocket_amd/score_model.py b/diffdock_pocket_amd/score_model.py
--- a/diffdock_pocket_amd/score_model.py
+++ b/diffdock_pocket_amd/score_model.py
@@ -418,6 +418,7 @@
         self._layer_specs, self._layer_specs_g = [], []
         self.factorize_min_degree = 3.0
         self.prune_last_receptor_layer = True
+        self.fused_front_lists = True
         self.share_layer0 = True
         self.share_clean_layer1 = True
         self.share_flex_layer0 = True
diff --git a/include/ddp_hip.h b/include/ddp_hip.h
--- a/include/ddp_hip.h
+++ b/include/ddp_hip.h
@@ -367,6 +367,64 @@
 } ddp_group_job_t;
 int ddp_group_by_key_jobs(const ddp_group_job_t* jobs, int njobs, void* stream);
 
+#define DDP_FRONT_MAX_LIG 64
+#define DDP_FRONT_MAX_REC 256
+#define DDP_FRONT_MAX_ATOM 2048
+#define DDP_FRONT_MAX_BONDS 256
+typedef struct {
+  int32_t* rowptr;
+  int32_t* perm;
+  int32_t* key;
+  int32_t* out0;
+  int32_t* out1;
+} ddp_front_view_t;
+typedef struct {
+  int32_t n_graphs;
+  int32_t n_lig, n_rec, n_atom, n_tor;
+  int32_t max_lig, max_rec, max_atom, max_tor, max_bonds;
+  const float* lig_pos;
+  const float* rec_pos;
+  const float* atom_pos;
+  const float* tor_pos;
+  const int32_t* lig_ptr;
+  const int32_t* rec_ptr;
+  const int32_t* atom_ptr;
+  const int32_t* tor_ptr;
+  float r_lig;
+  float r_cross;
+  const float* cross_div;
+  int32_t ll_neighbors, tor_neighbors, cross_neighbors, la_neighbors;
+  int32_t radius_flags;
+  int32_t e_bond;
+  int32_t* ll0;
+  int32_t* ll1;
+  int32_t cap_ll;
+  int32_t* cnt_ll;
+  int32_t* lr0;
+  int32_t* lr1;
+  int32_t cap_lr;
+  int32_t* cnt_lr;
+  int32_t* la0;
+  int32_t* la1;
+  int32_t cap_la;
+  int32_t* cnt_la;
+  int32_t* overflow;
+  int32_t* tor_q;
+  int32_t* tor_x;
+  int32_t cap_tor;
+  int32_t* cnt_tor;
+  int32_t* touched;
+  int32_t* near_rows;
+  int32_t* cnt_near;
+  int32_t* rp_lr;
+  int32_t* rp_la;
+  int32_t* rp_tor;
+  ddp_front_view_t c_ll, c_la, c_lr;
+  ddp_front_view_t so_ll, so_la, so_lr;
+  int32_t* scratch;
+} ddp_front_lists_t;
+int ddp_front_lists(const ddp_front_lists_t* a, int32_t* taken, void* stream);
+
 #define DDP_MAX_NODE_JOBS 8
 #define DDP_MAX_NODE_CAT 16
 typedef struct {
```

Result: faster. 181.1 (median of 6 runs) (+1.4%).
